# Funatiq/cuclark

Hardware: AMD Instinct MI355X
Metric: Mreads/sec (10M x 150bp, k=31) (higher is better)
Workload: dtype u64

## Files before the change

cuclark_amd/_lib.py:

```python
import ctypes as C
import importlib.util
import os
import subprocess

_PKG = os.path.dirname(os.path.abspath(__file__))
LIB_PATH = os.environ.get("MIC_LIB_PATH") or os.path.join(_PKG, "lib", "libmi_clark.so")
CSRC = os.path.join(_PKG, "csrc")

MIC_RESULT_WORDS = 8
MIC_FLAG_ROW_OVERFLOW = 1
MIC_FLAG_DENSE_PATH = 2
MIC_ROW_INVALID = 0xFFFFFFFF
MIC_ROLLUP_WORDS, MIC_ROLLUP_MAX_LEVELS = 8, 7
MIC_ROLLUP_UNRESOLVED, MIC_ROLLUP_PENDING = 0xFFFFFFFF, 0xFFFFFFFE
MIC_LAYOUT_AUTO, MIC_LAYOUT_DIRECT, MIC_LAYOUT_MINIMIZER, MIC_LAYOUT_SUPER, MIC_LAYOUT_SUPER2 = 0, 1, 2, 3, 4


class MicError(RuntimeError):
    def __init__(self, code, msg):
        super().__init__(f"libmi_clark error {code}: {msg}")
        self.code = code


class MicConfig(C.Structure):
    _fields_ = [("device", C.c_int32), ("k", C.c_int32), ("num_targets", C.c_uint32), ("num_batches", C.c_uint32),
                ("row_words", C.c_uint32), ("layout", C.c_uint32)]


class MicDbInfo(C.Structure):
    _fields_ = [("htsize", C.c_uint64), ("shard_start", C.c_uint64), ("shard_end", C.c_uint64),
                ("n_elems", C.c_uint64), ("n_elems_file", C.c_uint64), ("n_slots", C.c_uint64),
                ("n_overflow", C.c_uint64), ("hbm_bytes", C.c_uint64), ("key_bytes", C.c_int32),
                ("slot_class", C.c_int32), ("max_bucket", C.c_uint32), ("sampling", C.c_uint32), ("layout", C.c_int32),
                ("minimizer_len", C.c_int32), ("max_chain", C.c_uint32), ("reserved", C.c_uint32), ("n_entries", C.c_uint64),
                ("part", C.c_uint32), ("n_parts", C.c_uint32), ("part_slot_lo", C.c_uint64), ("part_slot_hi", C.c_uint64),
                ("n_slots_whole", C.c_uint64), ("side_kmers", C.c_uint64), ("side_bytes", C.c_uint64)]


class MicSynthSpec(C.Structure):
    _fields_ = [("seed", C.c_uint64), ("htsize", C.c_uint64), ("genome_nt", C.c_uint64), ("n_targets", C.c_uint32),
                ("n_genomes", C.c_uint32), ("k", C.c_int32), ("key_bytes", C.c_int32), ("keep_ppm", C.c_uint32), ("run_len", C.c_uint32),
                ("repeat_ppm", C.c_uint32), ("mosaic_ppm", C.c_uint32)]


class MicIngestResult(C.Structure):
    _fields_ = [("n_reads", C.c_uint64), ("csv_bytes", C.c_uint64), ("csv", C.c_void_p), ("results", C.c_void_p),
                ("status", C.c_uint32), ("n_lines", C.c_uint32)]


MIC_INGEST_OK, MIC_INGEST_FALLBACK, MIC_INGEST_ODD_RECORD, MIC_INGEST_TRUNCATED = 0, 1, 2, 4
MIC_INGEST_LONG_READ, MIC_INGEST_TOO_MANY, MIC_INGEST_DENSE = 8, 16, 32
MIC_INGEST_NO_CSV = 16


class MicAbundFilter(C.Structure):
    _fields_ = [("conf_num", C.c_uint64), ("conf_den", C.c_uint64), ("gamma_num", C.c_uint64), ("gamma_den", C.c_uint64)]

_VP, _SZ, _U32P, _U16P, _U64P = C.c_void_p, C.c_size_t, C.c_void_p, C.c_void_p, C.c_void_p
SYMBOLS = [
    ("mic_create", C.c_int, [C.POINTER(MicConfig), C.POINTER(_VP)]),
    ("mic_destroy", C.c_int, [_VP]),
    ("mic_last_error", C.c_char_p, []),
    ("mic_device_count", C.c_int, [C.POINTER(C.c_int)]),
    ("mic_db_load_files", C.c_int, [_VP, C.c_char_p, C.c_int, C.c_uint32, C.c_uint64, C.c_uint64]),
    ("mic_db_load_host", C.c_int, [_VP, _VP, C.c_uint64, _VP, C.c_int, _VP, C.c_uint32, C.c_uint64, C.c_uint64]),
    ("mic_db_load_device", C.c_int, [_VP, _VP, C.c_uint64, _VP, C.c_int, _VP, C.c_uint32, C.c_uint64, C.c_uint64]),
    ("mic_db_set_part", C.c_int, [_VP, C.c_uint32, C.c_uint32]),
    ("mic_db_reserve_hbm", C.c_int, [_VP, C.c_uint64]),
    ("mic_peer_matrix", C.c_int, [C.POINTER(C.c_int), C.c_int]),
    ("mic_device_memory", C.c_int, [C.c_int, C.POINTER(C.c_uint64), C.POINTER(C.c_uint64)]),
    ("mic_db_load_files_multi", C.c_int, [C.POINTER(C.c_void_p), _SZ, C.c_char_p, C.c_int, C.c_uint32]),
    ("mic_db_kernel_name", C.c_int, [_VP, C.c_char_p, _SZ]),
    ("mic_db_get_info", C.c_int, [_VP, C.POINTER(MicDbInfo)]),
    ("mic_db_unload", C.c_int, [_VP]),
    ("mic_db_last_build_report", C.c_char_p, []),
    ("mic_batches_alloc", C.c_int, [_VP, _SZ, _SZ, _SZ, _U32P, C.c_int, C.POINTER(_VP), C.POINTER(_VP), C.POINTER(_VP),
                                    C.POINTER(_VP)]),
    ("mic_batch_ready", C.c_int, [_VP, _SZ, _SZ, _SZ]),
    ("mic_batch_query", C.c_int, [_VP, _SZ, C.c_int, C.c_int]),
    ("mic_batch_wait", C.c_int, [_VP, _SZ]),
    ("mic_batch_dense_counts", C.c_int, [_VP, _SZ, _SZ, _VP]),
    ("mic_batch_check", C.c_int, [_VP, _SZ, C.POINTER(C.c_int)]),
    ("mic_batch_merge_shards", C.c_int, [C.POINTER(C.c_void_p), _SZ, _SZ]),
    ("mic_batch_query_group", C.c_int, [C.POINTER(C.c_void_p), _SZ, _SZ, C.c_int]),
    ("mic_sync", C.c_int, [_VP]),
    ("mic_thread_bind_near_device", C.c_int, [_VP, C.c_int]),
    ("mic_batches_free", C.c_int, [_VP]),
    ("mic_query_device", C.c_int, [_VP, _VP, _VP, _SZ, _VP, _VP, _VP]),
    ("mic_resolve_flagged_device", C.c_int, [_VP, _VP, _VP, _VP, _VP, _VP, C.POINTER(_SZ)]),
    ("mic_merge_rows_device", C.c_int, [_VP, _VP, _VP, _VP, _SZ, _VP]),
    ("mic_result_from_rows_device", C.c_int, [_VP, _VP, _VP, _SZ, _VP]),
    ("mic_count_dense_device", C.c_int, [_VP, _VP, _VP, _VP, _SZ, _VP, _VP]),
    ("mic_result_from_dense_device", C.c_int, [_VP, _VP, _VP, _SZ, _VP, _VP, _VP]),
    ("mic_probe_stats_device", C.c_int, [_VP, _VP, _VP, _SZ, C.POINTER(C.c_uint64)]),
    ("mic_last_query_ms", C.c_int, [_VP, C.POINTER(C.c_float)]),
    ("mic_last_crowd_stats", C.c_int, [_VP, C.POINTER(C.c_uint32)]),
    ("mic_debug_fetch_crowd", C.c_int, [_VP, _VP, _SZ, C.POINTER(C.c_uint32)]),
    ("mic_debug_stream_pool", C.c_int, [C.POINTER(C.c_uint32)]),
    ("mic_ingest_alloc", C.c_int, [_VP, _SZ, _SZ, C.POINTER(C.c_char_p), C.c_uint32, C.c_int, C.POINTER(_VP)]),
    ("mic_ingest_classify", C.c_int, [_VP, _SZ, _SZ, C.c_int, C.POINTER(MicIngestResult)]),
    ("mic_ingest_classify_group", C.c_int, [C.POINTER(C.c_void_p), _SZ, _SZ, _SZ, _SZ, C.c_int, C.POINTER(MicIngestResult)]),
    ("mic_ingest_fetch_group_rows", C.c_int, [_VP, _SZ, _SZ, _VP, _SZ, C.POINTER(C.c_uint64), C.POINTER(C.c_uint32)]),
    ("mic_ingest_group_stats", C.c_int, [_VP, C.POINTER(C.c_double), _SZ]),
    ("mic_ingest_fetch_packed", C.c_int, [_VP, _SZ, _VP, _SZ, _VP, _SZ, C.POINTER(C.c_uint64), C.POINTER(C.c_uint64)]),
    ("mic_ingest_free", C.c_int, [_VP]),
    ("mic_gz_inflate_device", C.c_int, [_VP, _VP, _SZ, C.POINTER(_VP), C.POINTER(_SZ), C.POINTER(C.c_uint32)]),
    ("mic_gz_copy_text", C.c_int, [_VP, _VP, _SZ, _SZ, _VP]),
    ("mic_gz_free_text", C.c_int, [_VP, _VP]),
    ("mic_gz_reserve", C.c_int, [_VP, _SZ, C.c_uint32]),
    ("mic_gz_reserve_bytes", C.c_uint64, [_SZ, C.c_uint32]),
    ("mic_gz_release", C.c_int, [_VP]),
    ("mic_pairs_index_device", C.c_int, [_VP, _VP, _SZ, _VP, _SZ, C.POINTER(_VP), C.POINTER(C.c_uint64), C.POINTER(C.c_uint32)]),
    ("mic_pairs_offsets", C.c_int, [_VP, C.POINTER(C.POINTER(C.c_uint64)), C.POINTER(_SZ), C.POINTER(C.c_uint32)]),
    ("mic_pairs_merge_to_slot", C.c_int, [_VP, _VP, C.c_uint64, C.c_uint64, _SZ, C.POINTER(_SZ)]),
    ("mic_pairs_text", C.c_int, [_VP, _VP, C.c_uint64, C.c_uint64, _VP, _SZ, C.POINTER(_SZ)]),
    ("mic_pairs_free", C.c_int, [_VP, _VP]),
    ("mic_text_index_device", C.c_int, [_VP, _VP, _SZ, C.POINTER(_VP), C.POINTER(C.c_uint64), C.POINTER(C.c_uint32)]),
    ("mic_text_index_front_device", C.c_int, [_VP, _VP, _SZ, C.POINTER(_VP), C.POINTER(C.c_uint64), C.POINTER(C.c_uint64), C.POINTER(C.c_uint32)]),
    ("mic_gz_stream_open", C.c_int, [_VP, _VP, _SZ, C.c_uint32, C.POINTER(_VP), C.POINTER(_VP), C.POINTER(_SZ)]),
    ("mic_gz_stream_next", C.c_int, [_VP, C.POINTER(_SZ), C.POINTER(C.c_int)]),
    ("mic_gz_stream_close", C.c_int, [_VP, C.c_int]),
    ("mic_text_offsets", C.c_int, [_VP, C.POINTER(C.POINTER(C.c_uint64)), C.POINTER(_SZ), C.POINTER(C.c_uint32)]),
    ("mic_text_to_slot", C.c_int, [_VP, _VP, C.c_uint64, C.c_uint64, _SZ, C.POINTER(_SZ)]),
    ("mic_text_copy", C.c_int, [_VP, _VP, C.c_uint64, C.c_uint64, _VP, _SZ, C.POINTER(_SZ)]),
    ("mic_text_free", C.c_int, [_VP, _VP]),
    ("mic_text_format", C.c_int, [_VP]),
    ("mic_abundance_start", C.c_int, [_VP, C.POINTER(MicAbundFilter)]),
    ("mic_abundance_fetch", C.c_int, [_VP, _VP, _SZ]),
    ("mic_abundance_stop", C.c_int, [_VP]),
    ("mic_abundance_device", C.c_int, [_VP, _VP, _VP, _SZ, C.POINTER(MicAbundFilter), _VP, _VP]),
    ("mic_abundance_host", C.c_int, [_VP, _VP, _SZ, C.c_int, C.c_uint32, C.POINTER(MicAbundFilter), _VP]),
    ("mic_abund_parse", C.c_int, [C.c_char_p, C.c_uint32, C.POINTER(C.c_uint64), C.POINTER(C.c_uint64)]),
    ("mic_rollup_check", C.c_int, [C.c_uint32, C.c_uint32, _VP]),
    ("mic_rollup_set", C.c_int, [_VP, C.c_uint32, _VP]),
    ("mic_rollup_layout", C.c_int, [_VP, _VP, C.POINTER(C.c_uint64)]),
    ("mic_rollup_device", C.c_int, [_VP, _VP, _VP, _SZ, C.POINTER(MicAbundFilter), _VP, _VP, _VP, _VP]),
    ("mic_rollup_dense_device", C.c_int, [_VP, _VP, _VP, _SZ, _VP, C.POINTER(MicAbundFilter), _VP, _VP, _VP, _VP]),
    ("mic_rollup_host", C.c_int, [_VP, C.c_uint32, _VP, _VP, _SZ, C.c_int, C.c_uint32, C.c_uint32, _VP, C.POINTER(MicAbundFilter),
                                  _VP, _VP, _VP]),
    ("mic_rollup_start", C.c_int, [_VP, C.POINTER(MicAbundFilter)]),
    ("mic_rollup_fetch", C.c_int, [_VP, _VP, _SZ]),
    ("mic_rollup_stop", C.c_int, [_VP]),
    ("mic_ingest_rollup_rows", C.c_int, [_VP, _SZ, C.POINTER(_VP), C.POINTER(C.c_uint64)]),
    ("mic_format_ratio_g", C.c_int, [C.c_uint32, C.c_uint32, C.c_char_p]),
    ("mic_key_bytes_rule", C.c_int, [C.c_uint64, C.c_int]),
    ("mic_index_reads", C.c_long, [_VP, _SZ, _SZ, _U64P, _U64P, _U64P, _U64P, _U64P]),
    ("mic_index_reads_parallel", C.c_long, [_VP, _SZ, C.c_int, _SZ, _U64P, _U64P, _U64P, _U64P, _U64P]),
    ("mic_find_record_start", _SZ, [_VP, _SZ, _SZ]),
    ("mic_find_record_start_in", _SZ, [_VP, _SZ, C.c_int, _SZ]),
    ("mic_pack_bound", _SZ, [_U64P, _U64P, _SZ, C.c_int]),
    ("mic_pack_reads", _SZ, [_VP, _U64P, _U64P, _U64P, _SZ, C.c_int, _U32P, _U16P, _SZ]),
    ("mic_csv_header", C.c_int, [C.c_char_p, _SZ, C.c_int, C.POINTER(C.c_char_p), C.c_uint32]),
    ("mic_csv_line", C.c_int, [C.c_char_p, _SZ, _VP, _SZ, C.c_uint64, C.c_int, C.c_int, _VP, C.POINTER(C.c_char_p),
                               C.c_uint32, C.c_int, _VP, _VP]),
    ("mic_db_build", C.c_int, [C.POINTER(C.c_char_p), _VP, _SZ, C.c_int, C.c_uint64, C.c_int, C.c_uint32, C.c_uint32, C.c_char_p,
                               C.c_int, C.c_int, C.c_uint32, C.POINTER(C.c_uint64)]),
    ("mic_db_build_error", C.c_char_p, []),
    ("mic_synth_db_device", C.c_int, [C.POINTER(MicSynthSpec), _VP, _VP, _VP, C.c_uint64, C.POINTER(C.c_uint64), _VP]),
    ("mic_synth_read_pitch", C.c_uint32, [C.c_uint32, C.c_int]),
    ("mic_synth_reads_device", C.c_int, [C.POINTER(MicSynthSpec), C.c_uint64, _SZ, C.c_uint32, C.c_double, C.c_double,
                                         C.c_double, _VP, _VP, _SZ, _VP, _VP]),
    ("mic_synth_reads_device2", C.c_int, [C.POINTER(MicSynthSpec), C.c_uint64, _SZ, C.c_uint32, C.c_int, C.c_double, C.c_double,
                                          C.c_double, _VP, _VP, _SZ, _VP, _VP]),
    ("mic_synth_text_record_bytes", _SZ, [C.c_uint32, C.c_int]),
    ("mic_synth_reads_text_device", C.c_int, [C.POINTER(MicSynthSpec), C.c_uint64, _SZ, C.c_uint32, C.c_double, C.c_double,
                                              C.c_double, C.c_int, C.c_int, _VP, _SZ, _VP]),
]

_lib = None


def build(verbose=False):
    r = subprocess.run(["make", "-C", CSRC, "all"], capture_output=True, text=True)
    if r.returncode != 0:
        raise RuntimeError("building libmi_clark.so failed:\n" + r.stdout[-4000:] + r.stderr[-4000:])
    if verbose:
        print(r.stdout)
    return LIB_PATH


def _share_hip_runtime_with_torch():
    if os.environ.get("MIC_NO_TORCH_HIP"):
        return
    try:
        spec = importlib.util.find_spec("torch")
    except Exception:
        spec = None
    if spec is None or not spec.origin:
        return
    p = os.path.join(os.path.dirname(spec.origin), "lib", "libamdhip64.so")
    if os.path.exists(p):
        try:
            C.CDLL(p, mode=C.RTLD_GLOBAL)
        except OSError:
            pass


def load():
    global _lib
    if _lib is not None:
        return _lib
    _share_hip_runtime_with_torch()
    if not os.path.exists(LIB_PATH):
        raise ImportError(f"{LIB_PATH} is missing: run `python -c 'import __graft_entry__ as g; g.build()'` "
                          "(there is no CPU fallback for the k-mer query path)")
    lib = C.CDLL(LIB_PATH)
    for name, res, args in SYMBOLS:
        fn = getattr(lib, name)
        fn.restype = res
        fn.argtypes = args
    _lib = lib
    return lib


def check(rc):
    if rc != 0:
        raise MicError(rc, load().mic_last_error().decode(errors="replace"))
```

cuclark_amd/csrc/mic_engine.hip:

```cpp
#include "mi_clark.h"
#include "mic_internal.h"

#include <errno.h>
#include <stdarg.h>
#include <stdio.h>
#include <stdlib.h>
#include <string.h>
#include <time.h>

#include <sched.h>

#include <algorithm>
#include <mutex>
#include <string>
#include <atomic>
#include <thread>
#include <unistd.h>
#include <utility>
#include <vector>

int mic_bind_thread_near_device(int device, int on);
bool mic_peer_enable(int from, int to);
void mic_peer_enable_engines(mic_engine* const* engines, size_t n);

// ... 36 lines not shown
  return he;
}

void mic_stream_put(hipStream_t s) {
  if (!s) return;
  (void)hipStreamSynchronize(s);
  StreamPool& P = pool();
  std::lock_guard<std::mutex> lk(P.mu);
  for (const auto& a : P.all_streams) if (a.second == s) { P.free_streams.push_back(a); return; }
}

hipError_t mic_event_get(hipEvent_t* ev, bool timing) {
  int dev = 0;
  hipError_t he = hipGetDevice(&dev);
  if (he != hipSuccess) return he;
  const int key = dev * 2 + (timing ? 1 : 0);
  StreamPool& P = pool();
  {
    std::lock_guard<std::mutex> lk(P.mu);
    for (size_t i = 0; i < P.free_events.size(); ++i)
      if (P.free_events[i].first == key) { *ev = P.free_events[i].second; P.free_events.erase(P.free_events.begin() + (ptrdiff_t)i); return hipSuccess; }
  }
  he = timing ? hipEventCreate(ev) : hipEventCreateWithFlags(ev, hipEventDisableTiming);
  if (he == hipSuccess) { std::lock_guard<std::mutex> lk(P.mu); P.all_events.emplace_back(key, *ev); }
  return he;
}

extern "C" int mic_debug_stream_pool(uint32_t out[4]) {
  if (!out) return MIC_E_INVALID;
  StreamPool& P = pool();
  std::lock_guard<std::mutex> lk(P.mu);
  out[0] = (uint32_t)P.all_streams.size(); out[1] = (uint32_t)P.free_streams.size();
  out[2] = (uint32_t)P.all_events.size(); out[3] = (uint32_t)P.free_events.size();
  return MIC_OK;
}

void mic_event_put(hipEvent_t ev) {
  if (!ev) return;
  (void)hipEventSynchronize(ev);
  StreamPool& P = pool();
  std::lock_guard<std::mutex> lk(P.mu);
  for (const auto& a : P.all_events) if (a.second == ev) { P.free_events.push_back(a); return; }
}
namespace {
std::mutex g_report_mu;
std::string g_report;
thread_local std::string t_report;

#define HIPTRY(x) do { hipError_t e_ = (x); if (e_ != hipSuccess) \
    return fail(e_ == hipErrorOutOfMemory ? MIC_E_NOMEM : MIC_E_HIP, "%s: %s", #x, hipGetErrorString(e_)); } while (0)

struct Batch {
  uint32_t* h_rp = nullptr; uint16_t* h_cont = nullptr;
  uint32_t* d_rp = nullptr; uint16_t* d_cont = nullptr;
  uint32_t* d_results = nullptr; uint32_t* d_rows = nullptr;
  uint32_t* d_flagged = nullptr; uint32_t* h_flagged = nullptr;
  uint32_t* d_peer = nullptr; uint32_t* d_acc = nullptr;
  uint32_t* d_crowd = nullptr;
  size_t first_read = 0, n_reads = 0, n_cont = 0, max_reads = 0, max_cont = 0;
  hipStream_t stream = nullptr;
  hipEvent_t done = nullptr, ev_up = nullptr, ev_k = nullptr;
  bool scheduled = false, resolved = true, extended = false;
};

}

struct mic_engine {
  mic_config cfg;
  int device = 0, n_cu = 256;
  hipStream_t stream = nullptr;
  hipStream_t up_stream = nullptr, down_stream = nullptr;
  bool db_loaded = false;
  uint4* slots = nullptr;
  uint4* side = nullptr;
  uint8_t* d_sizes = nullptr;
  MicTable table;
  int slot_class = 32;
  mic_db_info info;
  std::vector<Batch> batches;
  void* h_block = nullptr; void* d_block = nullptr;
  uint32_t* h_results = nullptr; uint32_t* h_rows = nullptr;
  size_t num_reads_total = 0;
  std::mutex submit_mu;
  uint32_t* d_flagged = nullptr; uint32_t flagged_cap = 0;
  uint32_t* d_crowd = nullptr; size_t crowd_reads = 0;
  hipEvent_t ev0 = nullptr, ev1 = nullptr;
  bool timed = false;
  size_t last_n_reads = 0;
  void* ingest = nullptr;
  uint64_t reserve_hbm = 0;
  uint32_t part = 0, n_parts = 0;
  MicAbund abund;
  MicRollup rollup;
};

namespace {

const uint32_t kFlaggedCap = 1u << 16;

int set_device(const mic_engine* e) {
  HIPTRY(hipSetDevice(e->device));
  return MIC_OK;
}

void fill_table(mic_engine* e, const MicBuildOut& b, uint64_t htsize, uint64_t s0, uint64_t s1, int key_bytes,
                uint32_t sampling, int layout, int m) {
  e->slots = b.slots;
  const bool parted = (layout == MIC_LAYOUT_SUPER || layout == MIC_LAYOUT_SUPER2) && (b.part_lo != 0 || b.part_hi != b.n_main);
  e->table.slots = parted ? b.slots - (ptrdiff_t)b.part_lo * 8 : b.slots;
  e->table.slot_lo = parted ? (uint32_t)b.part_lo : 0; e->table.slot_cnt = parted ? (uint32_t)(b.part_hi - b.part_lo) : 0;
  e->table.parted = parted ? 1 : 0;
  e->side = b.side;
  e->table.side = b.side; e->table.side_mask = b.side ? (uint32_t)(b.side_cells - 1) : 0;
  e->table.n_main = b.n_main;
  e->table.shard_start = s0;
  e->table.shard_end = s1;
  e->table.div = mic_make_div(htsize);
  e->table.k = e->cfg.k;
  e->table.layout = layout == MIC_LAYOUT_MINIMIZER ? 1 : (layout == MIC_LAYOUT_SUPER || layout == MIC_LAYOUT_SUPER2) ? 2 : 0;
  e->table.fwd = layout == MIC_LAYOUT_SUPER2 ? 1 : 0;
  e->table.m = m;
  e->table.sharded = (s0 != 0 || s1 != htsize) ? 1 : 0;
  e->table.sizes = e->d_sizes;
  mic_db_info& i = e->info;
  i.htsize = htsize; i.shard_start = s0; i.shard_end = s1;
  i.n_elems = b.n_elems; i.n_elems_file = b.n_elems_file;
  const uint64_t n_res = parted ? b.part_hi - b.part_lo : b.n_main;
  i.n_slots = n_res + b.n_overflow; i.n_overflow = b.n_overflow;
  i.part = e->n_parts > 1 ? e->part : 0; i.n_parts = e->n_parts > 1 ? e->n_parts : 0;
  i.part_slot_lo = parted ? b.part_lo : 0; i.part_slot_hi = parted ? b.part_hi : 0; i.n_slots_whole = b.n_main;
  i.side_kmers = b.side ? b.side_kmers : 0; i.side_bytes = b.side ? b.side_cells * 16 : 0;
  i.hbm_bytes = (b.side ? b.side_cells * 16 : 0) + (b.alloc_slots ? b.alloc_slots : n_res + b.n_overflow + 1) * (uint64_t)(layout != MIC_LAYOUT_DIRECT ? MIC_MSLOT_BYTES : MIC_SLOT_BYTES);
  i.key_bytes = key_bytes; i.slot_class = layout != MIC_LAYOUT_DIRECT ? 128 : e->slot_class; i.max_bucket = b.max_bucket;
  i.sampling = sampling; i.layout = layout; i.minimizer_len = layout != MIC_LAYOUT_DIRECT ? m : 0;
  i.max_chain = layout != MIC_LAYOUT_DIRECT ? b.max_chain : 0; i.reserved = (layout == MIC_LAYOUT_SUPER || layout == MIC_LAYOUT_SUPER2) ? b.walk_ppm : 0;
  i.n_entries = b.n_entries ? b.n_entries : b.n_elems;
  e->db_loaded = true;
  (void)mic_kernels_warm(e->stream);
}

int check_shard(uint64_t htsize, uint64_t& s0, uint64_t& s1) {
  if (htsize < 2 || htsize > 0xFFFFFFF0ULL) return fail(MIC_E_INVALID, "unsupported table size %llu", (unsigned long long)htsize);
  if (s1 == 0) s1 = htsize;
  if (s0 >= s1 || s1 > htsize) return fail(MIC_E_INVALID, "bad shard [%llu,%llu) of %llu", (unsigned long long)s0,
                                           (unsigned long long)s1, (unsigned long long)htsize);
  return MIC_OK;
}

struct UploadDst { int device; void* dst; hipStream_t stream; uint64_t lo, hi; };
struct UploadStage {
  static constexpr size_t CH = 256u << 20;
  void* buf[2] = {nullptr, nullptr};
  bool get(int near_device) {
    if (buf[0] && buf[1]) return true;
    mic_bind_thread_near_device(near_device, 1);
    bool ok = true;
    for (void*& b : buf) if (!b && ok) { ok = hipHostMalloc(&b, CH, hipHostMallocDefault) == hipSuccess; if (!ok) b = nullptr; }
    if (!ok) for (void*& b : buf) if (b) { hipHostFree(b); b = nullptr; }
    mic_bind_thread_near_device(near_device, 0);
    return ok;
  }
  ~UploadStage() { for (void* b : buf) if (b) hipHostFree(b); }
};
int upload_file_range_multi(FILE* f, const std::vector<UploadDst>& dsts, const char* what, UploadStage* shared = nullptr) {
  const size_t CH = UploadStage::CH;
  const int fd = fileno(f);
  static const int n_readers = [] { const char* e = getenv("MIC_LOAD_THREADS"); int v = e ? atoi(e) : 0; return v > 0 ? (v > 64 ? 64 : v) : 8; }();
// ... 327 lines not shown
void** mic_engine_ingest_slot(mic_engine* e) { return &e->ingest; }
MicAbund* mic_engine_abund(mic_engine* e) { return &e->abund; }
MicRollup* mic_engine_rollup(mic_engine* e) { return &e->rollup; }
uint32_t mic_engine_row_words(const mic_engine* e) { return e->cfg.row_words; }
hipStream_t mic_engine_stream(mic_engine* e) { return e->stream; }
void mic_engine_copy_streams(mic_engine* e, hipStream_t* up, hipStream_t* down) { *up = e->up_stream; *down = e->down_stream; }

void mic_build_report_add(const char* what, double seconds) {
  char line[256];
  snprintf(line, sizeof(line), "%s: %.4f\n", what, seconds);
  t_report += line;
}

namespace {
std::mutex g_peer_mu;
signed char g_peer[64][64];
}
bool mic_peer_enable(int from, int to) {
  if (from == to) return true;
  if (from < 0 || to < 0 || from >= 64 || to >= 64) return false;
  std::lock_guard<std::mutex> lk(g_peer_mu);
  if (g_peer[from][to]) return g_peer[from][to] > 0;
  int can = 0, cur = 0;
  hipGetDevice(&cur);
  bool ok = false;
  if (hipDeviceCanAccessPeer(&can, from, to) == hipSuccess && can && hipSetDevice(from) == hipSuccess) {
    const hipError_t he = hipDeviceEnablePeerAccess(to, 0);
    ok = he == hipSuccess || he == hipErrorPeerAccessAlreadyEnabled;
    (void)hipGetLastError();
  }
  hipSetDevice(cur);
  g_peer[from][to] = ok ? 1 : -1;
  return ok;
}
void mic_peer_enable_engines(mic_engine* const* engines, size_t n) {
  for (size_t i = 0; i < n; ++i)
    for (size_t j = 0; j < n; ++j)
      if (engines[i] && engines[j] && engines[i]->device != engines[j]->device) mic_peer_enable(engines[i]->device, engines[j]->device);
}

extern "C" {

const char* mic_last_error(void) { return g_err; }

int mic_device_count(int* count) {
  int n = 0;
  hipError_t e = hipGetDeviceCount(&n);
  if (e != hipSuccess) { *count = 0; return fail(MIC_E_NODEVICE, "hipGetDeviceCount: %s", hipGetErrorString(e)); }
  *count = n;
  return MIC_OK;
}

int mic_create(const mic_config* cfg, mic_engine** out) {
  if (!cfg || !out) return fail(MIC_E_INVALID, "null argument");
  if (cfg->k < 2 || cfg->k > 32) return fail(MIC_E_INVALID, "The k-mer length should be in [2,32].");
  if (cfg->num_targets > 65535) return fail(MIC_E_INVALID, "too many targets (%u > 65535)", cfg->num_targets);
  if (cfg->layout > MIC_LAYOUT_SUPER2) return fail(MIC_E_INVALID, "unknown table layout %u", cfg->layout);
  int n = 0;
  if (hipGetDeviceCount(&n) != hipSuccess || n == 0)
    return fail(MIC_E_NODEVICE, "no HIP device available: the MI355X engine cannot run (there is no CPU fallback)");
  int dev = cfg->device;
  if (dev < 0) { if (hipGetDevice(&dev) != hipSuccess) dev = 0; }
  if (dev >= n) return fail(MIC_E_INVALID, "device %d out of range (%d devices)", dev, n);
  hipDeviceProp_t prop;
  HIPTRY(hipSetDevice(dev));
  HIPTRY(hipGetDeviceProperties(&prop, dev));
  if (strncmp(prop.gcnArchName, "gfx950", 6) != 0)
    return fail(MIC_E_NODEVICE, "device %d is %s; this library carries gfx950 (MI355X) code objects only", dev, prop.gcnArchName);
  mic_engine* e = new (std::nothrow) mic_engine();
  if (!e) return fail(MIC_E_NOMEM, "out of host memory");
  e->cfg = *cfg;
  if (e->cfg.num_batches == 0) e->cfg.num_batches = 1;
  if (e->cfg.row_words == 0) e->cfg.row_words = 16;
  if (e->cfg.row_words < 2) e->cfg.row_words = 2;
  e->device = dev;
  e->n_cu = prop.multiProcessorCount;
  memset(&e->info, 0, sizeof(e->info));
  memset(&e->table, 0, sizeof(e->table));
  hipError_t he = mic_stream_get(&e->stream);
  if (he == hipSuccess) he = mic_stream_get(&e->up_stream);
  if (he == hipSuccess) he = mic_stream_get(&e->down_stream);
  if (he == hipSuccess) he = mic_event_get(&e->ev0, true);
  if (he == hipSuccess) he = mic_event_get(&e->ev1, true);
  if (he == hipSuccess) he = hipMalloc(&e->d_flagged, (size_t)(kFlaggedCap + 1) * 4);
  if (he != hipSuccess) { mic_destroy(e); return fail(MIC_E_HIP, "engine setup: %s", hipGetErrorString(he)); }
  e->flagged_cap = kFlaggedCap;
  *out = e;
  return MIC_OK;
}

int mic_destroy(mic_engine* e) {
  if (!e) return MIC_OK;
  hipSetDevice(e->device);
  hipDeviceSynchronize();
  mic_ingest_free(e);
  mic_gz_release(e);
  free_batches(e);
  if (e->slots) hipFree(e->slots);
  if (e->side) hipFree(e->side);
  if (e->d_sizes) hipFree(e->d_sizes);
  if (e->d_flagged) hipFree(e->d_flagged);
  if (e->d_crowd) hipFree(e->d_crowd);
  if (e->abund.d_counts) hipFree(e->abund.d_counts);
  if (e->rollup.d_counts) hipFree(e->rollup.d_counts);
  if (e->rollup.d_block) hipFree(e->rollup.d_block);
  if (e->ev0) mic_event_put(e->ev0);
  if (e->ev1) mic_event_put(e->ev1);
  if (e->stream) mic_stream_put(e->stream);
  if (e->up_stream) mic_stream_put(e->up_stream);
  if (e->down_stream) mic_stream_put(e->down_stream);
  delete e;
  return MIC_OK;
}

int mic_db_unload(mic_engine* e) {
  if (!e) return fail(MIC_E_INVALID, "null engine");
  int rc = set_device(e);
  if (rc) return rc;
  hipDeviceSynchronize();
  if (e->slots) hipFree(e->slots);
  if (e->side) hipFree(e->side);
  if (e->d_sizes) hipFree(e->d_sizes);
  e->slots = nullptr; e->side = nullptr; e->d_sizes = nullptr; e->db_loaded = false;
  memset(&e->info, 0, sizeof(e->info));
  return MIC_OK;
}

int mic_db_get_info(const mic_engine* e, mic_db_info* info) {
  if (!e || !info) return fail(MIC_E_INVALID, "null argument");
  if (!e->db_loaded) return fail(MIC_E_STATE, "no database loaded");
  *info = e->info;
  return MIC_OK;
}

const char* mic_db_last_build_report(void) {
  static thread_local std::string copy;
  std::lock_guard<std::mutex> lk(g_report_mu);
  copy = g_report;
  return copy.c_str();
}

int mic_db_reserve_hbm(mic_engine* e, uint64_t bytes) {
  if (!e) return fail(MIC_E_INVALID, "null engine");
  e->reserve_hbm = bytes;
  return MIC_OK;
}

int mic_db_set_part(mic_engine* e, uint32_t part, uint32_t n_parts) {
  if (!e) return fail(MIC_E_INVALID, "null engine");
  if (n_parts > 1 && part >= n_parts) return fail(MIC_E_INVALID, "part %u of %u", part, n_parts);
  if (n_parts > 65536) return fail(MIC_E_INVALID, "too many parts");
  if (e->db_loaded) return fail(MIC_E_STATE, "set the part before the database is loaded");
  e->part = n_parts > 1 ? part : 0; e->n_parts = n_parts > 1 ? n_parts : 0;
  return MIC_OK;
}

int mic_db_load_device(mic_engine* e, const uint8_t* d_sizes, uint64_t htsize, const void* d_keys, int key_bytes,
                       const uint16_t* d_labels, uint32_t sampling, uint64_t s0, uint64_t s1) {
  if (!e || !d_sizes || !d_keys || !d_labels) return fail(MIC_E_INVALID, "null argument");
  if (key_bytes != 2 && key_bytes != 4 && key_bytes != 8) return fail(MIC_E_INVALID, "key_bytes must be 2, 4 or 8");
  int rc = set_device(e);
  if (rc) return rc;
  if ((rc = check_shard(htsize, s0, s1))) return rc;
  if ((rc = apply_part(e, htsize, s0, s1))) return rc;
  if (e->db_loaded) mic_db_unload(e);
  uint64_t base_elems = 0, base_rank = 0;
  if (s0 > 0 && mic_reduce_sizes(d_sizes, s0, &base_elems, &base_rank, e->stream) != 0)
    return fail(MIC_E_HIP, "size reduction failed");
  return build_from_device(e, d_sizes + s0, htsize, s0, s1, (const char*)d_keys + base_elems * key_bytes, key_bytes,
                           d_labels + base_elems, sampling, base_rank);
}

int mic_db_load_host(mic_engine* e, const uint8_t* sizes, uint64_t htsize, const void* keys, int key_bytes,
                     const uint16_t* labels, uint32_t sampling, uint64_t s0, uint64_t s1) {
  if (!e || !sizes || !keys || !labels) return fail(MIC_E_INVALID, "null argument");
  if (key_bytes != 2 && key_bytes != 4 && key_bytes != 8) return fail(MIC_E_INVALID, "key_bytes must be 2, 4 or 8");
  int rc = set_device(e);
  if (rc) return rc;
  if ((rc = check_shard(htsize, s0, s1))) return rc;
  if ((rc = apply_part(e, htsize, s0, s1))) return rc;
  if (e->db_loaded) mic_db_unload(e);
  uint64_t base_elems = 0, base_rank = 0, n_el = 0;
  for (uint64_t i = 0; i < s0; ++i) { base_elems += sizes[i]; base_rank += sizes[i] > 0; }
  for (uint64_t i = s0; i < s1; ++i) n_el += sizes[i];
// ... 451 lines not shown
    std::vector<std::string> msgs(devs.size());
    std::vector<std::thread> th;
    for (size_t d = 0; d < devs.size(); ++d)
      th.emplace_back([&, d] {
        Dev& dv = devs[d];
        struct timespec ta; clock_gettime(CLOCK_MONOTONIC, &ta);
        for (size_t i : dv.eng) {
          mic_engine* e = engines[i];
          int r = set_device(e);
          if (!r) r = build_from_device(e, dv.d_sz + (er[i].s0 - dv.lo), htsize, er[i].s0, er[i].s1,
                                        (const char*)dv.d_ky + (er[i].base_elems - dv.el_lo) * key_bytes, key_bytes,
                                        dv.d_lb + (er[i].base_elems - dv.el_lo), sampling, er[i].base_rank);
          if (r) { rcs[d] = r; msgs[d] = g_err; break; }
        }
        hipSetDevice(dv.device);
        if (dv.d_sz) { hipFree(dv.d_sz); dv.d_sz = nullptr; }
        if (dv.d_ky) { hipFree(dv.d_ky); dv.d_ky = nullptr; }
        if (dv.d_lb) { hipFree(dv.d_lb); dv.d_lb = nullptr; }
        struct timespec tb; clock_gettime(CLOCK_MONOTONIC, &tb);
        dv.build_s = (tb.tv_sec - ta.tv_sec) + (tb.tv_nsec - ta.tv_nsec) / 1e9;
      });
    for (auto& t : th) t.join();
    for (size_t d = 0; d < devs.size(); ++d) if (rcs[d]) { rc = fail(rcs[d], "%s", msgs[d].c_str()); break; }
    if (timing)
      for (Dev& dv : devs) fprintf(stderr, "[load x%zu] device %d: %zu table(s) built in %.3f s\n", n_engines, dv.device, dv.eng.size(), dv.build_s);
    lap("tables built");
  } while (0);
  if (fs) fclose(fs);
  if (fk) fclose(fk);
  if (fl) fclose(fl);
  free(h_sz);
  for (Dev& dv : devs) {
    hipSetDevice(dv.device);
    if (dv.d_sz) hipFree(dv.d_sz);
    if (dv.d_ky) hipFree(dv.d_ky);
    if (dv.d_lb) hipFree(dv.d_lb);
  }
  return rc;
}

int mic_batch_check(mic_engine* e, size_t batch, int* done) {
  if (!e || batch >= e->batches.size() || !done) return fail(MIC_E_INVALID, "bad argument");
  Batch& B = e->batches[batch];
  if (!B.scheduled) { *done = 0; return MIC_OK; }
  hipError_t he = hipEventQuery(B.done);
  if (he == hipSuccess) *done = 1;
  else if (he == hipErrorNotReady) *done = 0;
  else return fail(MIC_E_HIP, "hipEventQuery: %s", hipGetErrorString(he));
  return MIC_OK;
}

int mic_thread_bind_near_device(mic_engine* e, int on) {
  if (!e) return fail(MIC_E_INVALID, "null engine");
  mic_bind_thread_near_device(e->device, on);
  return MIC_OK;
}

int mic_sync(mic_engine* e) {
  if (!e) return fail(MIC_E_INVALID, "null engine");
  int rc = set_device(e);
  if (rc) return rc;
  HIPTRY(hipDeviceSynchronize());
  return MIC_OK;
}

int mic_batches_free(mic_engine* e) {
  if (!e) return fail(MIC_E_INVALID, "null engine");
  int rc = set_device(e);
  if (rc) return rc;
  hipDeviceSynchronize();
  free_batches(e);
  return MIC_OK;
}

int mic_query_device(mic_engine* e, const uint32_t* d_rp, const uint16_t* d_cont, size_t n_reads, uint32_t* d_results,
                     uint32_t* d_rows, void* stream) {
  if (!e || !d_rp || !d_cont || !d_results) return fail(MIC_E_INVALID, "null argument");
  if (!e->db_loaded) return fail(MIC_E_STATE, "no database loaded");
  if (n_reads > 0xFFFFFFF0ull) return fail(MIC_E_INVALID, "too many reads in one call");
  if (((uintptr_t)d_cont & 3) || ((uintptr_t)d_rp & 3)) return fail(MIC_E_INVALID, "d_containers and d_reads_pointer must be 4-byte aligned");
  int rc = set_device(e);
  if (rc) return rc;
  hipStream_t s = stream ? (hipStream_t)stream : e->stream;
  HIPTRY(hipMemsetAsync(e->d_flagged, 0, 4, s));
  MicQueryArgs a;
  a.t = e->table; a.reads_ptr = d_rp; a.cont = d_cont; a.n_reads = (uint32_t)n_reads;
  a.row_words = e->cfg.row_words; a.results = d_results; a.rows = d_rows;
  a.flagged = e->d_flagged; a.flagged_cap = e->flagged_cap;
  if (e->table.side && n_reads > e->crowd_reads) {
    HIPTRY(hipStreamSynchronize(s));
    if (e->d_crowd) { hipFree(e->d_crowd); e->d_crowd = nullptr; e->crowd_reads = 0; }
    HIPTRY(hipMalloc(&e->d_crowd, mic_crowd_dims(n_reads).words * 4));
    e->crowd_reads = n_reads;
  }
  mic_crowd_attach(a, e->table.side ? e->d_crowd : nullptr, e->crowd_reads);
  HIPTRY(hipEventRecord(e->ev0, s));
  HIPTRY(mic_launch_query(a, e->slot_class, e->n_cu, s));
  HIPTRY(hipEventRecord(e->ev1, s));
  e->timed = true;
  e->last_n_reads = n_reads;
  return MIC_OK;
}

int mic_last_query_ms(mic_engine* e, float* ms) {
  if (!e || !ms) return fail(MIC_E_INVALID, "null argument");
  if (!e->timed) return fail(MIC_E_STATE, "no query was launched");
  HIPTRY(hipEventSynchronize(e->ev1));
  HIPTRY(hipEventElapsedTime(ms, e->ev0, e->ev1));
  return MIC_OK;
}

int mic_last_crowd_stats(mic_engine* e, uint32_t out[4]) {
  if (!e || !out) return fail(MIC_E_INVALID, "null argument");
  out[0] = out[1] = out[2] = out[3] = 0;
  if (!e->timed || !e->d_crowd || !e->table.side) return MIC_OK;
  int rc = set_device(e);
  if (rc) return rc;
  HIPTRY(hipEventSynchronize(e->ev1));
  HIPTRY(hipMemcpy(out, e->d_crowd, 16, hipMemcpyDeviceToHost));
  return MIC_OK;
}

int mic_debug_fetch_crowd(mic_engine* e, uint32_t* out, size_t words, uint32_t caps[3]) {
  if (!e || !out || !caps) return fail(MIC_E_INVALID, "null argument");
  if (!e->d_crowd || !e->timed) return fail(MIC_E_STATE, "no work area");
  int rc = set_device(e);
  if (rc) return rc;
  const MicCrowdDims d = mic_crowd_dims(e->crowd_reads);
  caps[0] = d.pend_cap; caps[1] = d.item_cap; caps[2] = d.pool_cap;
  HIPTRY(hipEventSynchronize(e->ev1));
  HIPTRY(hipMemcpy(out, e->d_crowd, (words < d.words ? words : d.words) * 4, hipMemcpyDeviceToHost));
  return MIC_OK;
}

int mic_resolve_flagged_device(mic_engine* e, const uint32_t* d_rp, const uint16_t* d_cont, uint32_t* d_results,
                               uint32_t* d_rows, void* stream, size_t* n_resolved) {
  if (!e || !d_rp || !d_cont || !d_results) return fail(MIC_E_INVALID, "null argument");
  int rc = set_device(e);
  if (rc) return rc;
  hipStream_t s = stream ? (hipStream_t)stream : e->stream;
  uint32_t nf = 0;
  HIPTRY(hipMemcpyAsync(&nf, e->d_flagged, 4, hipMemcpyDeviceToHost, s));
  HIPTRY(hipStreamSynchronize(s));
  if (n_resolved) *n_resolved = nf;
  if (!nf) return MIC_OK;
  if (nf > e->flagged_cap) {
    if (n_resolved) *n_resolved = e->last_n_reads;
    return run_dense(e, d_rp, d_cont, nullptr, e->last_n_reads, d_results, d_rows, s);
  }
  return run_dense(e, d_rp, d_cont, e->d_flagged + 1, nf, d_results, d_rows, s);
}

int mic_merge_rows_device(mic_engine* e, const uint32_t* a, const uint32_t* b, uint32_t* out, size_t n, void* stream) {
  if (!e || !a || !b || !out) return fail(MIC_E_INVALID, "null argument");
  int rc = set_device(e);
  if (rc) return rc;
  HIPTRY(mic_launch_merge_rows(a, b, out, e->cfg.row_words, n, nullptr, stream ? (hipStream_t)stream : e->stream));
  return MIC_OK;
}

int mic_result_from_rows_device(mic_engine* e, const uint32_t* rows, uint32_t* results, size_t n, void* stream) {
  if (!e || !rows || !results) return fail(MIC_E_INVALID, "null argument");
  int rc = set_device(e);
  if (rc) return rc;
  HIPTRY(mic_launch_result_from_rows(rows, e->cfg.row_words, results, n, stream ? (hipStream_t)stream : e->stream));
  return MIC_OK;
}

int mic_result_from_dense_device(mic_engine* e, const uint32_t* d_counts, const uint32_t* d_ids, size_t n_ids, uint32_t* d_results,
                                 uint32_t* d_rows, void* stream) {
  if (!e || !d_counts || !d_results) return fail(MIC_E_INVALID, "null argument");
  int rc = set_device(e);
  if (rc) return rc;
  HIPTRY(mic_launch_dense_finish(d_counts, d_ids, n_ids, e->cfg.num_targets ? e->cfg.num_targets : 1, d_results, d_rows,
                                 e->cfg.row_words, stream ? (hipStream_t)stream : e->stream));
  return MIC_OK;
}

int mic_probe_stats_device(mic_engine* e, const uint32_t* d_rp, const uint16_t* d_cont, size_t n_reads, uint64_t out[4]) {
  if (!e || !d_rp || !d_cont || !out) return fail(MIC_E_INVALID, "null argument");
  if (!e->db_loaded) return fail(MIC_E_STATE, "no database loaded");
  int rc = set_device(e);
  if (rc) return rc;
  unsigned long long* d = nullptr;
  unsigned long long h[4] = {0, 0, 0, 0};
  HIPTRY(hipMalloc(&d, 32));
  hipError_t he = hipMemsetAsync(d, 0, 32, e->stream);
  if (he == hipSuccess) he = mic_launch_probe_stats(e->table, e->slot_class, d_rp, d_cont, n_reads, d, e->stream);
  if (he == hipSuccess) he = hipMemcpyAsync(h, d, 32, hipMemcpyDeviceToHost, e->stream);
  if (he == hipSuccess) he = hipStreamSynchronize(e->stream);
  hipFree(d);
  if (he != hipSuccess) return fail(MIC_E_HIP, "probe stats: %s", hipGetErrorString(he));
  for (int i = 0; i < 4; ++i) out[i] = h[i];
  return MIC_OK;
}

int mic_count_dense_device(mic_engine* e, const uint32_t* d_rp, const uint16_t* d_cont, const uint32_t* d_ids,
                           size_t n_ids, uint32_t* d_counts, void* stream) {
  if (!e || !d_rp || !d_cont || !d_counts) return fail(MIC_E_INVALID, "null argument");
  if (!e->db_loaded) return fail(MIC_E_STATE, "no database loaded");
  int rc = set_device(e);
  if (rc) return rc;
// ... 7 lines not shown
```

cuclark_amd/csrc/mic_internal.h:

```cpp
#ifndef MIC_INTERNAL_H
#define MIC_INTERNAL_H

#include <hip/hip_runtime.h>
#include <stdint.h>
#include <stddef.h>

#include "mi_clark.h"

struct MicDiv {
  uint64_t d;
  uint64_t magic;
  uint32_t shift;
  uint32_t add;
};

MicDiv mic_make_div(uint64_t d);

#ifdef __cplusplus
#include <vector>
size_t mic_pack_reads_runs(const uint8_t* map, const uint64_t* seq_s, const uint64_t* seq_e, const uint64_t* length,
                           size_t n_reads, int k, uint32_t* reads_pointer, uint16_t* containers, size_t cap,
                           std::vector<uint64_t>* run_off, std::vector<uint64_t>* run_len);
#endif

static inline __host__ __device__ uint64_t mic_mulhi64(uint64_t a, uint64_t b) {
#if defined(__HIP_DEVICE_COMPILE__)
  return __umul64hi(a, b);
#else
  return (uint64_t)(((unsigned __int128)a * b) >> 64);
#endif
}

static inline __host__ __device__ uint64_t mic_div(uint64_t n, const MicDiv& dv) {
  if (dv.magic == 0) return n >> dv.shift;
  uint64_t t = mic_mulhi64(dv.magic, n);
  if (dv.add) return (((n - t) >> 1) + t) >> dv.shift;
  return t >> dv.shift;
}

#define MIC_SLOT_BYTES 64
#define MIC_FLAG_ROW_OVERFLOW_ 1u
#define MIC_FLAG_DENSE_PATH_ 2u
#define MIC_ROW_INVALID 0xFFFFFFFFu
#define MIC_CAP32 8
#define MIC_CAP64 4

#define MIC_MCAP 12
#define MIC_MSLOT_BYTES 128
#ifndef MIC_LAYOUT_MINIMIZER
#define MIC_LAYOUT_AUTO 0
#define MIC_LAYOUT_DIRECT 1
#define MIC_LAYOUT_MINIMIZER 2
#endif
#ifndef MIC_LAYOUT_SUPER
#define MIC_LAYOUT_SUPER 3
#endif
#ifndef MIC_LAYOUT_SUPER2
#define MIC_LAYOUT_SUPER2 4
#endif

struct MicTable {
  const uint4* slots;
  uint64_t n_main;
  uint64_t shard_start;
  uint64_t shard_end;
  MicDiv div;
  int k;
  int layout;
  int m;
  int sharded;
  int fwd;
  uint32_t slot_lo, slot_cnt;
  const uint4* side; uint32_t side_mask;
  int parted;
  const uint8_t* sizes;
};

struct MicQueryArgs {
  MicTable t;
  const uint32_t* reads_ptr;
  const uint16_t* cont;
  uint32_t n_reads;
  uint32_t row_words;
  uint32_t* results;
  uint32_t* rows;
  uint32_t* flagged;
  uint32_t flagged_cap;
  uint32_t* crowd;
  uint32_t* crowd_items; uint32_t* crowd_pool;
  uint32_t crowd_pend_cap, crowd_item_cap, crowd_pool_cap;
};

#define MIC_CROWD_HDR 8
#define MIC_CG_NONE 0xFFFFFFFFu
#define MIC_CG_DENSE 0xFFFFFFFEu
struct MicCrowdDims { uint32_t pend_cap, item_cap, pool_cap; size_t words; };
static inline MicCrowdDims mic_crowd_dims(size_t max_reads) {
  MicCrowdDims d;
  const size_t cap27 = (1u << 27) - 64;
  size_t pend = max_reads / 4 + 1024, item = max_reads + 4096, pool = max_reads * 2 + 8192;
  d.pend_cap = (uint32_t)(pend < cap27 ? pend : cap27);
  d.item_cap = (uint32_t)(item < cap27 ? item : cap27);
  d.pool_cap = (uint32_t)(pool < 0xFFFFFF00u ? pool : 0xFFFFFF00u);
  d.words = MIC_CROWD_HDR + 8 * ((size_t)d.pend_cap + d.item_cap) + d.pool_cap;
  return d;
}
static inline void mic_crowd_attach(MicQueryArgs& a, uint32_t* area, size_t max_reads) {
  const MicCrowdDims d = mic_crowd_dims(max_reads);
  a.crowd = area; a.crowd_pend_cap = area ? d.pend_cap : 0; a.crowd_item_cap = area ? d.item_cap : 0; a.crowd_pool_cap = area ? d.pool_cap : 0;
  a.crowd_items = area ? area + MIC_CROWD_HDR + 8 * (size_t)d.pend_cap : nullptr;
  a.crowd_pool = area ? a.crowd_items + 8 * (size_t)d.item_cap : nullptr;
}

void mic_build_report_add(const char* what, double seconds);
extern thread_local uint64_t mic_build_reserved_hbm;

hipError_t mic_launch_query(const MicQueryArgs& a, int slot_class, int n_cu, hipStream_t s);
int mic_query_kernel_name(const MicTable& t, int slot_class, char* buf, size_t cap);
hipError_t mic_kernels_warm(hipStream_t s);
hipError_t mic_launch_merge_rows(const uint32_t* a, const uint32_t* b, uint32_t* out, uint32_t row_words, size_t n,
                                 uint32_t* flags_results, hipStream_t s);
hipError_t mic_launch_result_from_rows(const uint32_t* rows, uint32_t row_words, uint32_t* results, size_t n,
                                       hipStream_t s);
hipError_t mic_launch_dense_count(const MicTable& t, int slot_class, const uint32_t* reads_ptr, const uint16_t* cont,
                                  const uint32_t* ids, size_t n_ids, uint32_t n_targets, uint32_t* counts,
                                  hipStream_t s);
hipError_t mic_launch_dense_finish(const uint32_t* counts, const uint32_t* ids, size_t n_ids, uint32_t n_targets,
                                   uint32_t* results, uint32_t* rows, uint32_t row_words, hipStream_t s);

hipError_t mic_launch_probe_stats(const MicTable& t, int slot_class, const uint32_t* reads_ptr, const uint16_t* cont,
                                  size_t n_reads, unsigned long long* d_out, hipStream_t s);

struct MicBuildOut {
  uint4* slots;
  uint64_t n_main, n_overflow, n_elems, n_elems_file;
  uint32_t max_bucket;
  uint32_t max_chain;
  uint32_t walk_ppm;
  uint64_t n_entries;
  uint4* side; uint64_t side_cells, side_kmers;
  uint64_t part_lo, part_hi;
  uint64_t alloc_slots;
};
int mic_build_table(const uint8_t* d_sizes, uint64_t n_buckets, const void* d_keys, int key_bytes,
                    const uint16_t* d_labels, uint32_t sampling, uint64_t rank_base, int slot_class, hipStream_t s,
                    MicBuildOut* out, char* err, size_t err_cap);
int mic_build_mtable(const uint8_t* d_sizes, uint64_t n_buckets, uint64_t bucket0, uint64_t htsize, const void* d_keys,
                     int key_bytes, const uint16_t* d_labels, uint32_t sampling, uint64_t rank_base, int k, int m,
                     hipStream_t s, MicBuildOut* out, char* err, size_t err_cap);
int mic_build_stable(const uint8_t* d_sizes, uint64_t n_buckets, uint64_t bucket0, uint64_t htsize, const void* d_keys,
                     int key_bytes, const uint16_t* d_labels, uint32_t sampling, uint64_t rank_base, int k, int m,
                     hipStream_t s, MicBuildOut* out, char* err, size_t err_cap, int allow_fallback, int both_strands,
                     uint32_t part, uint32_t n_parts);
int mic_reduce_sizes(const uint8_t* d_sizes, uint64_t n, uint64_t* total, uint64_t* nonzero, hipStream_t s);

hipError_t mic_stream_get(hipStream_t* s);
void mic_stream_put(hipStream_t s);
hipError_t mic_event_get(hipEvent_t* ev, bool timing);
void mic_event_put(hipEvent_t ev);

struct MicAbund {
  unsigned long long* d_counts = nullptr;
  uint32_t n_words = 0;
  bool on = false;
  uint64_t conf_num = 5, conf_den = 10, gamma_num = 0, gamma_den = 1;
};
hipError_t mic_launch_abund(const uint32_t* results, const uint32_t* norm, uint32_t norm_sub, size_t n, int k, uint32_t n_targets,
                            const MicAbund& f, unsigned long long* counts, const uint32_t* status, hipStream_t s);

struct MicRollup {
  uint32_t n_levels = 0;
  uint32_t n_groups[8] = {};
  uint32_t off[8] = {};
  uint32_t seg_off[8] = {};
  uint32_t n_counters = 0;
  void* d_block = nullptr;
  const uint16_t* d_group_of = nullptr;
  const uint16_t* d_perm = nullptr;
  const uint32_t* d_seg = nullptr;
  unsigned long long* d_counts = nullptr;
  bool on = false;
  mic_abund_filter filter = {5, 10, 0, 1};
};
hipError_t mic_launch_rollup(const MicRollup& ru, const uint32_t* rows, uint32_t row_words, const uint32_t* norm, uint32_t norm_sub, size_t n,
                             int k, uint32_t n_targets, const mic_abund_filter& f, uint32_t* rollup, uint32_t* levels,
                             unsigned long long* counts, const uint32_t* status, hipStream_t s);

#endif
```

cuclark_amd/csrc/mic_kernels.hip:

```cpp
#include "mic_internal.h"
#include "mic_device.h"

#include <stdlib.h>

#ifndef MIC_EXP
#define MIC_EXP 0
#endif
#ifndef MIC_FUNNEL64
#define MIC_FUNNEL64 1
#endif
#ifndef MIC_X
#define MIC_X 0
#endif

namespace {

__device__ __forceinline__ uint4 load_slot_quarter(const uint4* p) {
  typedef unsigned int u4 __attribute__((ext_vector_type(4)));
  u4 t = __builtin_nontemporal_load((const u4*)p);
  return make_uint4(t.x, t.y, t.z, t.w);
}

__device__ __forceinline__ uint64_t kmer_from_dwords(uint32_t d0, uint32_t d1, uint32_t d2, int nt_in_dword, int k) {
  const int s = 2 * nt_in_dword;
  uint64_t a = ((uint64_t)d0 << 32) | d1;
#if MIC_FUNNEL64
  uint64_t x = (a << s) | ((uint64_t)d2 >> (32 - s));
#else
  uint64_t x = s ? ((a << s) | (uint64_t)(d2 >> (32 - s))) : a;
#endif
  return x >> (64 - 2 * k);
}


struct ReadAhead { uint32_t pp, pe, hdr, w; };

__device__ __forceinline__ void ahead_ptr(const MicQueryArgs& a, uint32_t r, ReadAhead& x) {
  if (r < a.n_reads) { x.pp = a.reads_ptr[r]; x.pe = a.reads_ptr[r + 1]; } else { x.pp = 0; x.pe = 0; }
}

__device__ __forceinline__ void ahead_window(const uint16_t* __restrict__ cont, uint32_t r, uint32_t n_reads, int lane,
                                             ReadAhead& x) {
  x.hdr = 0; x.w = 0;
  if (r < n_reads) {
    const uint32_t pp = __builtin_amdgcn_readfirstlane(x.pp);
    x.hdr = cont[pp];
    if (lane < 10) x.w = ((uint32_t)cont[pp + 1 + 2 * lane] << 16) | cont[pp + 2 + 2 * lane];
  }
}

__device__ __forceinline__ uint32_t window_word(const uint16_t* __restrict__ cont, uint32_t first, uint32_t cend,
                                                uint32_t base, int lane, bool use_ahead, const ReadAhead& x) {
  uint32_t w = 0;
  const uint32_t ci = first + base / 8 + 2 * lane;
  if (use_ahead) w = x.w;
  else if (lane < 10) w = ((ci < cend ? (uint32_t)cont[ci] : 0u) << 16) | (ci + 1 < cend ? (uint32_t)cont[ci + 1] : 0u);
  if (lane >= 10 || ci >= cend) w &= 0x0000FFFFu;
  if (lane >= 10 || ci + 1 >= cend) w &= 0xFFFF0000u;
  return w;
}

__device__ __forceinline__ uint32_t window_word_w(const uint16_t* __restrict__ cont, uint32_t first, uint32_t cend,
                                                  uint32_t base, int lane, bool use_ahead, uint32_t ahead_w) {
  uint32_t w = 0;
  const uint32_t ci = first + base / 8 + 2 * lane;
  if (use_ahead) w = ahead_w;
  else if (lane < 10) w = ((ci < cend ? (uint32_t)cont[ci] : 0u) << 16) | (ci + 1 < cend ? (uint32_t)cont[ci + 1] : 0u);
  if (lane >= 10 || ci >= cend) w &= 0x0000FFFFu;
  if (lane >= 10 || ci + 1 >= cend) w &= 0xFFFF0000u;
  return w;
}

struct Probe {
  uint32_t slot;
  uint32_t qlo, qhi;
};

template <bool KEY64>
__device__ __forceinline__ Probe make_probe(const MicTable& t, uint64_t kmer, bool active) {
  uint64_t c = canonical(kmer, t.k);
  uint64_t q = mic_div(c, t.div);
  uint64_t rem = c - q * t.div.d;
  Probe p;
  bool ok = active && rem >= t.shard_start && rem < t.shard_end;
  if (!KEY64) ok = ok && (q >> 32) == 0;
  p.slot = ok ? (uint32_t)(rem - t.shard_start) : 0xFFFFFFFFu;
// ... 146 lines not shown
    }
  }
}

template <bool KEY64>
__global__ void __launch_bounds__(256) query_kernel(const MicQueryArgs a) {
  const int lane = threadIdx.x & 63;
  const int j = lane & 3;
  const uint32_t wave0 = __builtin_amdgcn_readfirstlane(blockIdx.x * 4 + (threadIdx.x >> 6));
  const uint32_t n_waves = gridDim.x * 4;
  const MicTable& t = a.t;
  const int k = t.k;
  const uint4* __restrict__ slots = t.slots;
  const uint16_t* __restrict__ cont = a.cont;

  for (uint32_t r = wave0; r < a.n_reads; r += n_waves) {
    ReadAhead cur;
    ahead_ptr(a, r, cur);
    ahead_window(cont, r, a.n_reads, lane, cur);
    uint32_t pp = __builtin_amdgcn_readfirstlane(cur.pp);
    const uint32_t pe = __builtin_amdgcn_readfirstlane(cur.pe);
    RowAcc acc; acc.label1 = 0; acc.count = 0;
    uint32_t n_ent = 0, overflow = 0, total = 0;
    bool first_part = true;

    while (pp < pe) {
      const uint32_t plen = __builtin_amdgcn_readfirstlane(first_part ? cur.hdr : (uint32_t)cont[pp]);
      const bool ahead_ok = first_part;
      first_part = false;
      if (plen == 0) break;
      const uint32_t first = pp + 1;
      pp = first + (plen + 7) / 8;
      if (plen < (uint32_t)k) continue;
      const uint32_t nk = plen - k + 1;
      const uint32_t cend = pp;
      for (uint32_t base = 0; base < nk; base += 128) {
        const uint32_t w = window_word(cont, first, cend, base, lane, ahead_ok && base == 0, cur);
        Probe pr[2];
#pragma unroll
        for (int h = 0; h < 2; ++h) {
          const int idx = 4 * h + (lane >> 4);
          uint32_t d0 = bperm(idx, w), d1 = bperm(idx + 1, w), d2 = bperm(idx + 2, w);
          uint64_t kmer = kmer_from_dwords(d0, d1, d2, lane & 15, k);
          pr[h] = make_probe<KEY64>(t, kmer, base + 64 * h + lane < nk);
        }
        uint4 q[8]; uint32_t qlo[8], qhi[8]; uint32_t sl[8];
#pragma unroll
        for (int s = 0; s < 8; ++s) {
          const int src = 16 * (s & 3) + (lane >> 2);
          sl[s] = bperm(src, pr[s >> 2].slot);
          qlo[s] = bperm(src, pr[s >> 2].qlo);
          qhi[s] = KEY64 ? bperm(src, pr[s >> 2].qhi) : 0;
          q[s] = make_uint4(0, 0, 0, 0);
          if (sl[s] != 0xFFFFFFFFu) q[s] = load_slot_quarter(slots + (uint64_t)sl[s] * 4 + j);
        }
        uint32_t res0 = 0, res1 = 0;
#pragma unroll
        for (int s = 0; s < 8; ++s) {
          uint32_t m = match_quarter<KEY64>(q[s], qlo[s], qhi[s], j);
          m |= quad_perm<QP_XOR1>(m);
          m |= quad_perm<QP_XOR2>(m);
          constexpr uint32_t CAP = KEY64 ? MIC_CAP64 : MIC_CAP32;
          if (__ballot((q[s].w & 0xFF) > CAP))
            m = chase_chain<KEY64>(slots, q[s], qlo[s], qhi[s], j, m, sl[s] != 0xFFFFFFFFu);
          if (s < 4) res0 = (j == (s & 3)) ? m : res0;
          else res1 = (j == (s & 3)) ? m : res1;
        }
        tally2(res0, res1, acc, n_ent, overflow, total, lane);
      }
    }
    finish_read(acc, n_ent, total, overflow, r, a, lane);
  }
}


#define MIC_RMAX 32
#define MIC_MSTRIDE 8
#ifndef MIC_R_SKEW
#define MIC_R_SKEW 2
#endif
#ifndef MIC_R_PIPE
#define MIC_R_PIPE 2
#endif
__device__ __forceinline__ uint32_t staged_at(uint32_t i) { return i * MIC_MSTRIDE + (i >> 3) * MIC_R_SKEW; }
#ifndef MIC_M_SKEW
#define MIC_M_SKEW 0
#endif
__device__ __forceinline__ uint32_t staged_at_m(uint32_t i) { return i * MIC_MSTRIDE + (i >> 3) * MIC_M_SKEW; }

__device__ __forceinline__ void sliding_min3(uint32_t& a0, uint32_t& a1, uint32_t& a2, int w, int lane) {
  auto step = [&](int s) {
    const int src = (lane + s) & 63;
    const bool wrap = lane + s >= 64;
    uint32_t x0 = bperm(src, a0), x1 = bperm(src, a1), x2 = bperm(src, a2);
    uint32_t n0 = wrap ? x1 : x0, n1 = wrap ? x2 : x1, n2 = wrap ? 0xFFFFFFFFu : x2;
    a0 = n0 < a0 ? n0 : a0; a1 = n1 < a1 ? n1 : a1; a2 = n2 < a2 ? n2 : a2;
  };
  int cover = 1;
  while (2 * cover <= w) { step(cover); cover *= 2; }
  if (cover < w) step(w - cover);
}

__device__ __forceinline__ void sliding_min2(uint32_t& a0, uint32_t& a1, int w, int lane) {
  auto step = [&](int s) {
    const int src = (lane + s) & 63;
    const bool wrap = lane + s >= 64;
    uint32_t x0 = bperm(src, a0), x1 = bperm(src, a1);
    uint32_t n0 = wrap ? x1 : x0, n1 = wrap ? 0xFFFFFFFFu : x1;
    a0 = n0 < a0 ? n0 : a0; a1 = n1 < a1 ? n1 : a1;
  };
  int cover = 1;
  while (2 * cover <= w) { step(cover); cover *= 2; }
  if (cover < w) step(w - cover);
}

__device__ __forceinline__ uint32_t row_prefix_min(uint32_t t) {
  uint32_t x;
  x = (uint32_t)__builtin_amdgcn_update_dpp(-1, (int)t, 0x111, 0xF, 0xF, false); t = x < t ? x : t;
  x = (uint32_t)__builtin_amdgcn_update_dpp(-1, (int)t, 0x112, 0xF, 0xF, false); t = x < t ? x : t;
  x = (uint32_t)__builtin_amdgcn_update_dpp(-1, (int)t, 0x114, 0xF, 0xF, false); t = x < t ? x : t;
  x = (uint32_t)__builtin_amdgcn_update_dpp(-1, (int)t, 0x118, 0xF, 0xF, false); t = x < t ? x : t;
  return t;
}

__device__ __forceinline__ uint32_t row_suffix_min(uint32_t t) {
  uint32_t x;
  x = (uint32_t)__builtin_amdgcn_update_dpp(-1, (int)t, 0x101, 0xF, 0xF, false); t = x < t ? x : t;
  x = (uint32_t)__builtin_amdgcn_update_dpp(-1, (int)t, 0x102, 0xF, 0xF, false); t = x < t ? x : t;
  x = (uint32_t)__builtin_amdgcn_update_dpp(-1, (int)t, 0x104, 0xF, 0xF, false); t = x < t ? x : t;
  x = (uint32_t)__builtin_amdgcn_update_dpp(-1, (int)t, 0x108, 0xF, 0xF, false); t = x < t ? x : t;
  return t;
}

template <int BANKS>
__device__ __forceinline__ uint32_t with_row_in_front(uint32_t P) {
  const uint32_t f = (uint32_t)__builtin_amdgcn_update_dpp(-1, (int)P, 0x142, 0xE, BANKS, false);
  return f < P ? f : P;
}
__device__ __forceinline__ void sliding_min_rows(uint32_t& a0, uint32_t& a1, uint32_t a2, int W, int lane, int lane_inv) {
  const uint32_t P0 = row_prefix_min(a0), P1 = row_prefix_min(a1), P2 = row_prefix_min(a2);
  if (W > 16 && ((W - 16) & 3) == 0) {
    const uint32_t S0 = row_suffix_min(a0), S1 = row_suffix_min(a1);
    const int s = W - 16, bm = (1 << (s >> 2)) - 1;
    uint32_t Q0, Q1, Q2;
    switch (bm) {
      case 1: Q0 = with_row_in_front<1>(P0); Q1 = with_row_in_front<1>(P1); Q2 = with_row_in_front<1>(P2); break;
      case 3: Q0 = with_row_in_front<3>(P0); Q1 = with_row_in_front<3>(P1); Q2 = with_row_in_front<3>(P2); break;
      case 7: Q0 = with_row_in_front<7>(P0); Q1 = with_row_in_front<7>(P1); Q2 = with_row_in_front<7>(P2); break;
      default: Q0 = with_row_in_front<15>(P0); Q1 = with_row_in_front<15>(P1); Q2 = with_row_in_front<15>(P2); break;
    }
    const uint32_t f0 = __builtin_amdgcn_readlane(P0, 63), f1 = __builtin_amdgcn_readlane(P1, 63);
    const bool head = lane < s;
    const uint32_t h1 = f0 < Q1 ? f0 : Q1, h2 = f1 < Q2 ? f1 : Q2;
    Q1 = head ? h1 : Q1; Q2 = head ? h2 : Q2;
    const int at = (lane_inv << 2) + ((W - 1) << 2);
    const uint32_t z0 = (uint32_t)__builtin_amdgcn_ds_bpermute(at, (int)Q0), z1 = (uint32_t)__builtin_amdgcn_ds_bpermute(at, (int)Q1),
                   z2 = (uint32_t)__builtin_amdgcn_ds_bpermute(at, (int)Q2);
    const bool wz = lane >= 65 - W;
    const uint32_t v0 = wz ? z1 : z0, v1 = wz ? z2 : z1;
    a0 = v0 < S0 ? v0 : S0; a1 = v1 < S1 ? v1 : S1;
    return;
  }
  const uint32_t S0 = row_suffix_min(a0), S1 = row_suffix_min(a1), S2 = row_suffix_min(a2);
  const int at = lane_inv << 2;
  const uint32_t x0 = (uint32_t)__builtin_amdgcn_ds_bpermute(at + 60, (int)P0), x1 = (uint32_t)__builtin_amdgcn_ds_bpermute(at + 60, (int)P1),
                 x2 = (uint32_t)__builtin_amdgcn_ds_bpermute(at + 60, (int)P2);
// ... 506 lines not shown
                const bool m1 = same1 && ((p1 >> (16 + (w - 1) - ao[1])) & 1) && s_extract(a1, b1, c1, (int)ao[1], k) == ko[1];
                if (m0) hit0 = (p0 & 0xFFFFu) + 1;
                if (m1) hit1 = (p1 & 0xFFFFu) + 1;
                {
                  const bool cr0 = same0 && (p0 >> 16) == 0, cr1 = same1 && (p1 >> 16) == 0;
                  if (__ballot(cr0) | __ballot(cr1)) {
                    uint64_t kp = (uint64_t)__builtin_amdgcn_kernarg_segment_ptr();
                    asm volatile("" : "+s"(kp));
                    const __attribute__((address_space(4))) MicQueryArgs* kc = (const __attribute__((address_space(4))) MicQueryArgs*)kp;
                    const uint4* side = kc->t.side; const uint32_t smask = kc->t.side_mask;
                    const uint64_t mm = (1ULL << (2 * m)) - 1;
                    if (side && cr0 && s_extract(a0, b0, c0, w - 1, m) == ((ko[0] >> (2 * ao[0])) & mm)) hit0 = s_side_probe(side, smask, ko[0]);
                    if (side && cr1 && s_extract(a1, b1, c1, w - 1, m) == ((ko[1] >> (2 * ao[1])) & mm)) hit1 = s_side_probe(side, smask, ko[1]);
                  }
                }
                more0 = same0 && !m0 && e0 < 5; more1 = same1 && !m1 && e1 < 5;
                e0 += more0 ? 1u : 0u; e1 += more1 ? 1u : 0u;
                if (!(__ballot(more0) | __ballot(more1))) break;
              }
              if (v0) { o0_ = hit0; y0_ = 0xFFFFFFFFu; }
              if (v1) { o1_ = hit1; y1_ = 0xFFFFFFFFu; }
              const bool n0 = v0 && !hit0 && (mz0 & MIC_S_NEXT), n1 = v1 && !hit1 && (mz1 & MIC_S_NEXT);
              if (__ballot(n0) | __ballot(n1)) {
                if (n0 && q0[5] <= t0) y0_ = q0[31];
                if (n1 && q1[5] <= t1) y1_ = q1[31];
              }
            }
          }
        };
        while (__ballot(sl0 != 0xFFFFFFFFu) | __ballot(sl1 != 0xFFFFFFFFu)) {
          uint32_t nx0, nx1;
          level(sl0, sl1, res0, res1, nx0, nx1);
          sl0 = nx0; sl1 = nx1;
        }
        tally2(res0, res1, acc, n_ent, overflow, total, lane);
      }
    }
    uint32_t t_hdr, t_pp, t_pe;
    asm volatile("s_waitcnt vmcnt(0)" ::: "memory");
    __builtin_amdgcn_wave_barrier();
    ahead_take(ahead_sel ? ahead1 : ahead0, n_pp, t_hdr, t_pp, t_pe);
    __builtin_amdgcn_wave_barrier();
    {
      uint64_t kp = (uint64_t)__builtin_amdgcn_kernarg_segment_ptr();
      asm volatile("" : "+s"(kp));
      const __attribute__((address_space(4))) MicQueryArgs* kc = (const __attribute__((address_space(4))) MicQueryArgs*)kp;
      struct { uint32_t* results; uint32_t* rows; uint32_t* flagged; uint32_t row_words, flagged_cap; } fa;
      fa.results = kc->results; fa.rows = kc->rows; fa.flagged = kc->flagged; fa.row_words = kc->row_words; fa.flagged_cap = kc->flagged_cap;
      finish_read(acc, n_ent, total, overflow, r, fa, lane);
    }
    ahead_issue(ahead_sel ? ahead0 : ahead1, t_pp, r + 3 * n_waves);
    ahead_sel ^= 1;
    cur_pp = n_pp; cur_pe = n_pe; cur_hdr = t_hdr; n_pp = t_pp; n_pe = t_pe;
  }
}


__device__ __forceinline__ uint64_t wballot(bool p) { return __builtin_amdgcn_ballot_w64(p); }

static_assert(MIC_RMAX <= 32, "tally_counts sums the first two rows of lanes");
#define MIC_R_CROWDED (-16)
__device__ __forceinline__ void tally_counts(uint32_t lab1, uint32_t cnt, RowAcc& acc, uint32_t& n_ent, uint32_t& overflow,
                                             uint32_t& total, int lane) {
  uint64_t mm = wballot(lab1 != 0);
  while (mm) {
    const uint32_t l1 = __builtin_amdgcn_readlane(lab1, __builtin_ctzll(mm));
    const bool mine = lab1 == l1;
    mm &= ~wballot(mine);
    const uint32_t c = mine ? cnt : 0u;
    uint32_t sum = 0;
    {
      uint32_t v = c;
      v += (uint32_t)__builtin_amdgcn_update_dpp(0, (int)v, 0x111, 0xF, 0xF, true);
      v += (uint32_t)__builtin_amdgcn_update_dpp(0, (int)v, 0x112, 0xF, 0xF, true);
      v += (uint32_t)__builtin_amdgcn_update_dpp(0, (int)v, 0x114, 0xF, 0xF, true);
      v += (uint32_t)__builtin_amdgcn_update_dpp(0, (int)v, 0x118, 0xF, 0xF, true);
      sum = __builtin_amdgcn_readlane(v, 15) + __builtin_amdgcn_readlane(v, 31);
    }
    total += sum;
    row_add(acc, n_ent, overflow, l1, sum, lane);
  }
}

template <int KK, int MM, bool FWD, bool PART>
__global__ void __launch_bounds__(64 * MIC_M_WPB, 32 / MIC_M_WPB) query_kernel_r(const MicQueryArgs a) {
  __shared__ uint4 s_stage[MIC_M_WPB][MIC_RMAX * MIC_MSTRIDE + (MIC_RMAX / 8 - 1) * MIC_R_SKEW];
  __shared__ uint16_t s_rec[MIC_M_WPB][132];
  __shared__ uint32_t s_ahead[MIC_M_WPB][2][64];
  __shared__ uint32_t s_part[PART ? MIC_M_WPB : 1][2];
  const int lane = threadIdx.x & 63;
  const int wv = __builtin_amdgcn_readfirstlane(threadIdx.x >> 6);
  uint4* stage = s_stage[wv];
  uint16_t* rec = s_rec[wv];
  const uint32_t wave0 = __builtin_amdgcn_readfirstlane(blockIdx.x * MIC_M_WPB + wv);
  const uint32_t n_waves = gridDim.x * MIC_M_WPB;
  const MicTable& t = a.t;
  if (PART) { if (lane == 0) { s_part[wv][0] = t.slot_lo; s_part[wv][1] = t.slot_cnt; } __builtin_amdgcn_wave_barrier(); }
  const int k = KK ? KK : t.k, m = MM ? MM : t.m, ctx = k - m;
  const uint4* __restrict__ slots = t.slots;
  const uint16_t* __restrict__ cont = a.cont;
  auto below = [](uint64_t mask) { return (uint32_t)__builtin_amdgcn_mbcnt_hi((uint32_t)(mask >> 32), __builtin_amdgcn_mbcnt_lo((uint32_t)mask, 0u)); };

  uint32_t* ahead0 = s_ahead[wv][0];
  uint32_t* ahead1 = s_ahead[wv][1];
  auto ahead_issue = [&](uint32_t* entry, uint32_t pp_w, uint32_t r_ptr) {
    const uint64_t abase = ((uint64_t)(cont + pp_w)) & ~3ULL;
    const uint32_t rr = r_ptr < a.n_reads ? r_ptr : a.n_reads - 1;
    const uint64_t pbase = (uint64_t)(a.reads_ptr + rr) - 48;
    int ln = lane;
    asm volatile("" : "+v"(ln));
    if (ln < 12)
      __builtin_amdgcn_global_load_lds((const __attribute__((address_space(1))) void*)((const uint32_t*)abase + lane),
                                       (__attribute__((address_space(3))) void*)entry, 4, 0, 0);
    uint64_t pb = pbase + 48;
    asm volatile("" : "+s"(pb));
    if (ln < 2)
      __builtin_amdgcn_global_load_lds((const __attribute__((address_space(1))) void*)((const uint32_t*)pb + lane),
                                       (__attribute__((address_space(3))) void*)(entry + 12), 4, 0, 0);
  };
  auto ahead_take = [&](const uint32_t* entry, uint32_t pp_w, uint32_t& hdr, uint32_t& npp, uint32_t& npe) {
    const uint32_t raw = entry[lane];
    npp = __builtin_amdgcn_readlane(raw, 12); npe = __builtin_amdgcn_readlane(raw, 13);
    const bool odd = (((uint64_t)(cont + pp_w)) >> 1) & 1;
    const uint32_t first = __builtin_amdgcn_readfirstlane(raw);
    hdr = odd ? first >> 16 : first & 0xFFFFu;
  };
  auto ahead_word = [&](const uint32_t* entry, uint32_t pp_w) {
    const uint32_t raw = entry[lane];
    const bool odd = (((uint64_t)(cont + pp_w)) >> 1) & 1;
    const uint32_t up = (uint32_t)__builtin_amdgcn_update_dpp(0, (int)raw, 0x101, 0xF, 0xF, true);
    return __builtin_amdgcn_perm(up, raw, odd ? 0x05040706u : 0x03020504u);
  };
  uint32_t cur_pp, cur_pe, cur_hdr, n_pp, n_pe, ahead_sel;
  {
    const uint32_t r0 = wave0 < a.n_reads ? wave0 : a.n_reads - 1;
    cur_pp = __builtin_amdgcn_readfirstlane(a.reads_ptr[r0]); cur_pe = __builtin_amdgcn_readfirstlane(a.reads_ptr[r0 + 1]);
    ahead_issue(ahead0, cur_pp, wave0 + n_waves);
    asm volatile("s_waitcnt vmcnt(0)" ::: "memory");
    __builtin_amdgcn_wave_barrier();
    ahead_take(ahead0, cur_pp, cur_hdr, n_pp, n_pe);
    ahead_issue(ahead1, n_pp, wave0 + 2 * n_waves);
    ahead_sel = 1;
  }
  constexpr bool PIPE = KK != 0 && (MIC_R_PIPE >= 2 || (MIC_R_PIPE == 1 && FWD));
  struct Round {
    uint32_t G0, G1, G2, cur;
    int jmax, jmin, remaining;
  };
  auto front = [&](const uint32_t first, const uint32_t cend, const uint32_t base, const uint32_t nk, const bool use_ahead, uint32_t& wd_out) __attribute__((always_inline)) -> uint32_t {
    int ln = lane;
    asm volatile("" : "+v"(ln));
    const uint32_t wd = use_ahead ? ahead_word(ahead_sel ? ahead0 : ahead1, cur_pp)
                                  : window_word_w(cont, first, cend, base, ln, false, 0u);
    wd_out = wd;
    const uint32_t n_act = nk - base < 128u ? nk - base : 128u;
    const bool past = n_act + (uint32_t)(k - s_tlen(k, m)) >= 129u;
    uint32_t qa0, qa1;
    sampled_positions<!FWD>(wd, ln, lane, k, m, past, qa0, qa1);
    qa0 = (uint32_t)lane < n_act ? qa0 : 0xFFu;
    qa1 = 64u + (uint32_t)lane < n_act ? qa1 : 0xFFu;
    const uint32_t last0 = __builtin_amdgcn_readlane(qa0, 63);
    uint32_t p0 = (uint32_t)__builtin_amdgcn_update_dpp(-1, (int)qa0, 0x138, 0xF, 0xF, false);
    uint32_t p1 = (uint32_t)__builtin_amdgcn_update_dpp((int)last0, (int)qa1, 0x138, 0xF, 0xF, false);
    const bool f0 = qa0 != p0, f1 = qa1 != p1;
    const uint64_t b0 = wballot(f0), b1 = wballot(f1);
    const uint32_t R0 = __popcll(b0), R = R0 + __popcll(b1) - (n_act < 128u ? 1u : 0u);
    __builtin_amdgcn_wave_barrier();
    if (f0) rec[below(b0)] = (uint16_t)(qa0 | ((uint32_t)lane << 8));
    if (f1) rec[R0 + below(b1)] = (uint16_t)(qa1 | ((64u + (uint32_t)lane) << 8));
    if (__builtin_expect(n_act == 128u, 0)) {
      asm volatile("" ::: "memory");
      if (ln == 0) rec[R] = (uint16_t)(128u << 8);
    }
    __builtin_amdgcn_wave_barrier();
    return R;
  };
  const uint32_t xsh = (64u - 2u * (uint32_t)k) & 31u;
  auto region_x = [&](uint32_t A0, uint32_t A1, uint32_t& lo, uint32_t& hi) {
    if (k > 16) {
      lo = __builtin_amdgcn_alignbit(A0, A1, xsh) & (m >= 16 ? 0xFFFFFFFFu : (1u << ((2 * m) & 31)) - 1u);
      hi = m > 16 ? (A0 >> xsh) & ((1u << ((2 * m - 32) & 31)) - 1u) : 0u;
    } else {
      const uint64_t x = ((((uint64_t)A0 << 32) | A1) << (2 * ctx)) >> (64 - 2 * m);
      lo = (uint32_t)x; hi = (uint32_t)(x >> 32);
    }
  };
  auto setup = [&](const uint32_t wd, const uint32_t rbase, const uint32_t R, Round& L, uint32_t& nrun_out) __attribute__((always_inline)) {
    const uint32_t nrun = R - rbase < MIC_RMAX ? R - rbase : MIC_RMAX;
    nrun_out = nrun;
    const bool vr = (uint32_t)lane < nrun;
    const uint32_t ri = vr ? rbase + (uint32_t)lane : 0u;
    const uint32_t rc0 = rec[ri], rc1 = rec[ri + 1];
    const int qa = (int)(rc0 & 255u), i0 = (int)(rc0 >> 8);
    const int n = (int)(rc1 >> 8) - i0;
    const int s1 = qa - ctx - 1;
    const int D = s1 >> 4;
    const uint32_t tsh = 30u - 2u * (uint32_t)(s1 & 15);
    const int a0 = D << 2;
    const uint32_t W0 = (uint32_t)__builtin_amdgcn_ds_bpermute(a0, (int)wd), W1 = (uint32_t)__builtin_amdgcn_ds_bpermute(a0 + 4, (int)wd),
                   W2 = (uint32_t)__builtin_amdgcn_ds_bpermute(a0 + 8, (int)wd), W3 = (uint32_t)__builtin_amdgcn_ds_bpermute(a0 + 12, (int)wd);
    uint32_t G0 = __builtin_amdgcn_alignbit(W0, W1, tsh), G1 = __builtin_amdgcn_alignbit(W1, W2, tsh), G2 = __builtin_amdgcn_alignbit(W2, W3, tsh);
    uint32_t key, xhi;
    region_x(G0, G1, key, xhi);
    bool rev = false;
    if (!FWD) {
      const uint32_t sh = 96u - 2u * (uint32_t)(k + ctx);
      const uint32_t r0 = __builtin_bitreverse32(G2), r1 = __builtin_bitreverse32(G1), r2 = __builtin_bitreverse32(G0);
      uint32_t q0 = sh ? __builtin_amdgcn_alignbit(r0, r1, 32u - sh) : r0;
      uint32_t q1 = sh ? __builtin_amdgcn_alignbit(r1, r2, 32u - sh) : r1;
      uint32_t q2 = r2 << sh;
      q0 = ~(((q0 >> 1) & 0x55555555u) | ((q0 << 1) & 0xAAAAAAAAu));
      q1 = ~(((q1 >> 1) & 0x55555555u) | ((q1 << 1) & 0xAAAAAAAAu));
      q2 = ~(((q2 >> 1) & 0x55555555u) | ((q2 << 1) & 0xAAAAAAAAu));
      uint32_t kr, hr;
      region_x(q0, q1, kr, hr);
      rev = hr < xhi || (hr == xhi && kr < key);
      G0 = rev ? q0 : G0; G1 = rev ? q1 : G1; G2 = rev ? q2 : G2;
      key = rev ? kr : key; xhi = rev ? hr : xhi;
    }
    const int jmaxf = qa - i0, jminf = jmaxf - n + 1;
    const int jmax = rev ? ctx - jminf : jmaxf, jmin = rev ? ctx - jmaxf : jminf;
    uint32_t cur = vr ? sslot_of_x32(key, xhi, (uint32_t)t.n_main) : 0xFFFFFFFFu;
    bool mine = vr;
    if (PART) {
      mine = vr && cur - s_part[wv][0] < s_part[wv][1];
      cur = mine ? cur : 0xFFFFFFFFu;
    }
    L.G0 = G0; L.G1 = G1; L.G2 = G2; L.cur = cur;
    L.jmax = jmax; L.jmin = jmin; L.remaining = mine ? n : 0;
  };
  auto issue = [&](const uint32_t cur, const uint32_t nrun) __attribute__((always_inline)) {
    uint32_t sidx[MIC_RMAX / 8];
    int ln = lane;
    asm volatile("" : "+v"(ln));
    __builtin_amdgcn_wave_barrier();
    if (ln < MIC_RMAX) ((uint32_t*)stage)[lane] = cur;
    __builtin_amdgcn_wave_barrier();
    uint32_t so = (uint32_t)(uintptr_t)(__attribute__((address_space(3))) void*)stage;
    asm volatile("" : "+s"(so));
#pragma unroll
    for (int i = 0; i < MIC_RMAX / 8; ++i) sidx[i] = ((const uint32_t*)stage)[8 * i + (lane >> 3)];
#pragma unroll
    for (int i = 0; i < MIC_RMAX / 8; ++i) {
      if (8u * i >= nrun) break;
      if (sidx[i] != 0xFFFFFFFFu)
        __builtin_amdgcn_global_load_lds((const __attribute__((address_space(1))) void*)(slots + (uint64_t)sidx[i] * 8 + (lane & 7)),
                                         (__attribute__((address_space(3))) void*)(uintptr_t)(so + 16u * (64 + MIC_R_SKEW) * (uint32_t)i), 16, 0, 0);
    }
  };
  auto consume = [&](Round& L, RowAcc& acc, uint32_t& n_ent, uint32_t& overflow, uint32_t& total, uint32_t& cg) __attribute__((always_inline)) {
    const uint32_t G0 = L.G0, G1 = L.G1, G2 = L.G2;
    uint32_t key, xhi_;
    region_x(G0, G1, key, xhi_);
    const int jmax = L.jmax, jmin = L.jmin;
    uint32_t cur = L.cur;
    int remaining = L.remaining;
    bool again = false;
    do {
      if (again) issue(cur, MIC_RMAX);
      again = true;
      asm volatile("s_waitcnt vmcnt(0)" ::: "memory");
      __builtin_amdgcn_wave_barrier();
      const bool vl = cur != 0xFFFFFFFFu;
      const uint32_t* q = (const uint32_t*)(stage + (vl ? staged_at((uint32_t)lane) : 0));
      const uint4 ka = *(const uint4*)q;
      const uint2 kb = *(const uint2*)(q + 4);
      uint32_t e = (ka.x < key) + (ka.y < key) + (ka.z < key) + (ka.w < key) + (kb.x < key) + (kb.y < key);
      const uint32_t mz = q[30];
      bool more = vl && e < 6;
      e = e < 5 ? e : 5;
      for (;;) {
        uint32_t e3 = e + (e << 1);
        asm volatile("" : "+v"(e3));
        uint32_t g = q[e], S0 = q[6 + e3], S1 = q[7 + e3], S2 = q[8 + e3], pl = q[24 + e];
        asm volatile("" : "+v"(S2));
        const bool same = more && g == key;
        const uint32_t d0 = G0 ^ S0, d1 = G1 ^ S1, d2 = G2 ^ S2;
        const bool mineq = k > 16
                               ? ((d0 & ((1u << ((32 - 2 * ctx) & 31)) - 1u)) | (d1 >> xsh)) == 0
                               : (((((uint64_t)d0 << 32) | d1) << (2 * ctx)) >> (64 - 2 * m)) == 0;
        const uint32_t dl = d0 >> (32 - 2 * ctx);
        const uint32_t dr = k > 16 ? __builtin_amdgcn_alignbit(d1, d2, xsh)
                                        : (uint32_t)((((((uint64_t)d0 << 32) | d1)) << ((2 * k) & 63)) >> 32);
        const int left = __builtin_ctz(dl | (1u << (2 * ctx))) >> 1;
        const int right = __builtin_clz(dr | (1u << (31 - 2 * ctx))) >> 1;
        const int hi = left < jmax ? left : jmax, lo = ctx - right > jmin ? ctx - right : jmin;
        const uint32_t range = ((2u << (hi & 31)) - 1u) & (~0u << (lo & 31));
        const uint32_t hits = (same && mineq) ? (uint32_t)__popc((pl >> 16) & range) : 0u;
#if !(MIC_X & 1)
        remaining = (same && mineq && (pl >> 16) == 0) ? MIC_R_CROWDED : remaining;
#endif
        const uint32_t lab_new = (pl & 0xFFFFu) + 1u;
        tally_counts(hits ? lab_new : 0u, hits, acc, n_ent, overflow, total, lane);
        remaining -= (int)hits;
        more = same && remaining > 0 && e < 5;
        e += more ? 1u : 0u;
        if (!wballot(more)) break;
      }
      const bool nx = vl && remaining > 0 && (mz & MIC_S_NEXT);
      cur = 0xFFFFFFFFu;
      if (wballot(nx)) { if (nx && q[5] <= key) cur = q[31]; }
    } while (wballot(cur != 0xFFFFFFFFu));
    if (!(MIC_X & 2) && __builtin_expect(wballot(remaining <= MIC_R_CROWDED) != 0, 0)) {
      const bool crowded = remaining <= MIC_R_CROWDED;
      const uint32_t n_c = (uint32_t)__popcll(wballot(crowded));
      uint64_t kpv = (uint64_t)__builtin_amdgcn_kernarg_segment_ptr();
      asm volatile("" : "+v"(kpv));
      const MicQueryArgs* kv = (const MicQueryArgs*)kpv;
      uint32_t* cw = kv->crowd;
      uint32_t* itb = kv->crowd_items;
      const uint32_t icap = kv->crowd_item_cap;
      uint32_t ib = 0xFFFFFFFFu;
      if (cw != nullptr && cg != MIC_CG_DENSE) {
        uint32_t v = 0;
        if (lane == 0) v = atomicAdd(&cw[1], n_c);
        ib = __builtin_amdgcn_readfirstlane(v);
      }
      asm volatile("" : "+v"(ib));
      const bool room = ib <= icap && n_c <= icap - ib;
      if (crowded && room) {
        uint32_t* it = itb + 8 * ((size_t)ib + below(wballot(crowded)));
        it[0] = G0; it[1] = G1; it[2] = G2; it[3] = (uint32_t)jmin | ((uint32_t)jmax << 8);
        it[4] = cg;
      }
      cg = __builtin_amdgcn_readfirstlane(room ? (ib | ((n_c - 1u) << 27)) : MIC_CG_DENSE);
    }
  };
  auto finish = [&](const RowAcc& acc, uint32_t n_ent, uint32_t total, uint32_t overflow, uint32_t r, const uint32_t cg) __attribute__((always_inline)) {
    uint32_t spilled = 0;
    if (!(MIC_X & 4) && __builtin_expect(cg != MIC_CG_NONE, 0)) {
      uint64_t kpv = (uint64_t)__builtin_amdgcn_kernarg_segment_ptr();
      asm volatile("" : "+v"(kpv));
      const MicQueryArgs* kv = (const MicQueryArgs*)kpv;
      uint32_t* cw = kv->crowd;
      uint32_t* pool = kv->crowd_pool;
      const uint32_t pcap = kv->crowd_pend_cap, wcap = kv->crowd_pool_cap;
      uint32_t p = 0xFFFFFFFFu, off = 0;
      if (cg != MIC_CG_DENSE) {
        if (lane == 0) { p = atomicAdd(&cw[0], 1u); off = atomicAdd(&cw[2], 2u * n_ent); }
        p = __builtin_amdgcn_readfirstlane(p); off = __builtin_amdgcn_readfirstlane(off);
      }
      asm volatile("" : "+v"(p), "+v"(off));
      const bool room = off <= wcap && 2u * n_ent <= wcap - off;
      if (p < pcap) {
        uint32_t* pd = cw + MIC_CROWD_HDR + 8 * (size_t)p;
        if (lane == 0) { pd[0] = r; pd[1] = total; pd[2] = room ? (n_ent | (overflow << 8)) : 0xFFFFFFFFu; pd[3] = off; pd[4] = cg; }
        if (room && (uint32_t)lane < n_ent) { uint32_t* pe_ = pool + (size_t)off + 2 * lane; pe_[0] = acc.label1; pe_[1] = acc.count; }
      }
      spilled = __builtin_amdgcn_readfirstlane((p < pcap && room) ? 1u : 0u);
      if (!spilled) {
        if (lane == 0 && cw != nullptr && cg != MIC_CG_DENSE) atomicAdd(&cw[3], 1u);
        overflow = 1;
      }
    }
    if (!spilled) {
      uint64_t kp = (uint64_t)__builtin_amdgcn_kernarg_segment_ptr();
      asm volatile("" : "+s"(kp));
      const __attribute__((address_space(4))) MicQueryArgs* kc = (const __attribute__((address_space(4))) MicQueryArgs*)kp;
      struct { uint32_t* results; uint32_t* rows; uint32_t* flagged; uint32_t row_words, flagged_cap; } fa;
      fa.results = kc->results; fa.rows = kc->rows; fa.flagged = kc->flagged; fa.row_words = kc->row_words; fa.flagged_cap = kc->flagged_cap;
      finish_read(acc, n_ent, total, overflow, r, fa, lane);
    }
  };

  uint32_t r = wave0; bool p_valid = false;
  auto step = [&](Round& P, Round& N) __attribute__((always_inline)) -> bool {
    const bool have = r < a.n_reads;
    uint32_t pp = cur_pp;
    const uint32_t pe = cur_pe;
    bool shape = false, simple = false;
    uint32_t n_nrun = 0, plen0 = 0, pp1 = 0;
    if (have) {
      plen0 = cur_hdr; pp1 = pp + 1 + (plen0 + 7) / 8;
      shape = plen0 - (uint32_t)k < 128u && pp1 == pe;
      if (!shape && plen0 - (uint32_t)k < 128u && pp1 < pe) {
        const uint32_t rel = pp1 - cur_pp + (uint32_t)((((uint64_t)(cont + cur_pp)) >> 1) & 1);
        if (rel < 24u) {
          const uint32_t v = (ahead_sel ? ahead0 : ahead1)[rel >> 1];
          shape = __builtin_amdgcn_readfirstlane((rel & 1u) ? v >> 16 : v & 0xFFFFu) == 0;
        }
      }
      if (PIPE && shape) {
        uint32_t n_wd;
        const uint32_t R = front(pp + 1, pp1, 0u, plen0 - (uint32_t)k + 1u, true, n_wd);
        if (R <= MIC_RMAX) { setup(n_wd, 0u, R, N, n_nrun); simple = true; }
      }
    }
    if (PIPE && p_valid) {
      RowAcc acc; acc.label1 = 0; acc.count = 0;
      uint32_t n_ent = 0, overflow = 0, total = 0, cg = MIC_CG_NONE;
      consume(P, acc, n_ent, overflow, total, cg);
      finish(acc, n_ent, total, overflow, r - n_waves, cg);
    } else {
      asm volatile("s_waitcnt vmcnt(0)" ::: "memory");
    }
    if (!have) return false;
    if (!simple) {
      RowAcc acc; acc.label1 = 0; acc.count = 0;
      uint32_t n_ent = 0, overflow = 0, total = 0, cg = MIC_CG_NONE;
      auto chunk = [&](const uint32_t first, const uint32_t cend, const uint32_t base, const uint32_t nk, const bool use_ahead) __attribute__((always_inline)) {
        uint32_t wd;
        const uint32_t R = front(first, cend, base, nk, use_ahead, wd);
        for (uint32_t rbase = 0; rbase < R; rbase += MIC_RMAX) {
          Round L; uint32_t nrun;
          setup(wd, rbase, R, L, nrun);
          issue(L.cur, nrun);
          consume(L, acc, n_ent, overflow, total, cg);
        }
      };
      if (!PIPE && shape) chunk(pp + 1, pp1, 0u, plen0 - (uint32_t)k + 1u, true);
      else {
        bool first_part = true;
        while (pp < pe) {
          uint32_t plen;
          {
            const uint32_t rel = pp - cur_pp + (uint32_t)((((uint64_t)(cont + cur_pp)) >> 1) & 1);
            if (first_part) plen = cur_hdr;
            else if (rel < 24u) {
              const uint32_t v = (ahead_sel ? ahead0 : ahead1)[rel >> 1];
              plen = __builtin_amdgcn_readfirstlane((rel & 1u) ? v >> 16 : v & 0xFFFFu);
            } else plen = __builtin_amdgcn_readfirstlane((uint32_t)cont[pp]);
          }
          const bool ahead_ok = first_part;
          first_part = false;
          if (plen == 0) break;
          const uint32_t first = pp + 1;
          pp = first + (plen + 7) / 8;
          if (plen < (uint32_t)k) continue;
          const uint32_t nk = plen - k + 1;
          const uint32_t cend = pp;
          for (uint32_t base = 0; base < nk; base += 128) chunk(first, cend, base, nk, ahead_ok && base == 0);
        }
      }
      finish(acc, n_ent, total, overflow, r, cg);
    }
    uint32_t t_hdr, t_pp, t_pe;
    __builtin_amdgcn_wave_barrier();
    ahead_take(ahead_sel ? ahead1 : ahead0, n_pp, t_hdr, t_pp, t_pe);
    __builtin_amdgcn_wave_barrier();
    ahead_issue(ahead_sel ? ahead0 : ahead1, t_pp, r + 3 * n_waves);
    ahead_sel ^= 1;
    cur_pp = n_pp; cur_pe = n_pe; cur_hdr = t_hdr; n_pp = t_pp; n_pe = t_pe;
    p_valid = simple;
    if (simple) issue(N.cur, n_nrun);
    r += n_waves;
    return true;
  };
  Round Ra, Rb;
  while (step(Ra, Rb) && step(Rb, Ra)) {}
}

__global__ void __launch_bounds__(256) crowd_finish_kernel(const MicQueryArgs a) {
  const int lane = threadIdx.x & 63;
  const uint32_t wave0 = __builtin_amdgcn_readfirstlane(blockIdx.x * 4 + (threadIdx.x >> 6)), n_waves = gridDim.x * 4;
  const uint32_t* __restrict__ cw = a.crowd;
  const uint32_t pcap = a.crowd_pend_cap;
  uint32_t np = cw[0];
  np = np < pcap ? np : pcap;
  const uint32_t* __restrict__ pend = cw + MIC_CROWD_HDR;
  const uint32_t* __restrict__ items = a.crowd_items;
  const uint32_t* __restrict__ pool = a.crowd_pool;
  const uint4* __restrict__ side = a.t.side;
  const uint32_t smask = a.t.side_mask;
  const int k = a.t.k, ctx = k - a.t.m;
  for (uint32_t p = wave0; p < np; p += n_waves) {
    const uint4 h = *(const uint4*)(pend + 8 * (size_t)p);
    const uint32_t r = __builtin_amdgcn_readfirstlane(h.x), meta = __builtin_amdgcn_readfirstlane(h.z), off = __builtin_amdgcn_readfirstlane(h.w);
    uint32_t total = __builtin_amdgcn_readfirstlane(h.y);
    uint32_t g = __builtin_amdgcn_readfirstlane(pend[8 * (size_t)p + 4]);
    if (meta == 0xFFFFFFFFu) continue;
    uint32_t n_ent = meta & 0xFFu, overflow = (meta >> 8) & 1u;
    RowAcc acc; acc.label1 = 0; acc.count = 0;
    if ((uint32_t)lane < n_ent) { const uint2 e = *(const uint2*)(pool + off + 2 * lane); acc.label1 = e.x; acc.count = e.y; }
    while (g != MIC_CG_NONE) {
      const uint32_t ib = g & 0x7FFFFFFu, n_c = (g >> 27) + 1u;
      g = __builtin_amdgcn_readfirstlane(items[8 * (size_t)ib + 4]);
      for (uint32_t b = 0; b < n_c; b += 4) {
        const uint32_t idx = b + ((uint32_t)lane >> 4);
        const bool valid = idx < n_c;
        uint4 it = make_uint4(0, 0, 0, 0);
        if (valid) it = *(const uint4*)(items + 8 * (size_t)(ib + idx));
        const int jmin = (int)(it.w & 0xFFu), jmax = (int)((it.w >> 8) & 0xFFu);
        int j = jmin + (lane & 15);
        bool go = valid && j <= jmax;
        j = go ? j : jmin;
        const uint64_t K = s_extract(it.x, it.y, it.z, ctx - j, k);
        uint32_t hsh = s_side_hash(K, smask), got = 0;
        while (wballot(go)) {
          uint4 c = make_uint4(0, 0, 0, 0);
          if (go) c = load_slot_quarter(side + hsh);
          if (go) {
            if (c.z == 0) go = false;
            else if (c.x == (uint32_t)K && c.y == (uint32_t)(K >> 32)) { got = c.z; go = false; }
            else hsh = (hsh + 1) & smask;
          }
        }
        tally2(got, 0u, acc, n_ent, overflow, total, lane);
      }
    }
    finish_read(acc, n_ent, total, overflow, r, a, lane);
  }
}


__global__ void merge_rows_kernel(const uint32_t* __restrict__ ra, const uint32_t* __restrict__ rb,
                                  uint32_t* __restrict__ out, uint32_t row_words, size_t n,
                                  uint32_t* __restrict__ results) {
  size_t i = (size_t)blockIdx.x * blockDim.x + threadIdx.x;
  if (i >= n) return;
  const uint32_t* a = ra + i * row_words; const uint32_t* b = rb + i * row_words; uint32_t* o = out + i * row_words;
  uint32_t na = a[0], nb = b[0], ia = 0, ib = 0, no = 0;
  bool ok = na != MIC_ROW_INVALID && nb != MIC_ROW_INVALID;
  if (!ok) { na = 0; nb = 0; }
  while (ia < na || ib < nb) {
    uint32_t va = ia < na ? a[1 + ia] : 0xFFFFFFFFu, vb = ib < nb ? b[1 + ib] : 0xFFFFFFFFu;
    uint32_t ta = ia < na ? (va & 0xFFFF) : 0x10000u, tb = ib < nb ? (vb & 0xFFFF) : 0x10000u;
    uint32_t tgt, cnt;
    if (ta < tb) { tgt = ta; cnt = va >> 16; ++ia; }
    else if (tb < ta) { tgt = tb; cnt = vb >> 16; ++ib; }
    else { tgt = ta; cnt = (va >> 16) + (vb >> 16); ++ia; ++ib; }
    if (no + 1 < row_words && cnt <= 0xFFFF) o[1 + no] = (cnt << 16) | tgt; else ok = false;
    ++no;
  }
  o[0] = ok ? no : MIC_ROW_INVALID;
  (void)results;
}

__global__ void result_rows_kernel(const uint32_t* __restrict__ rows, uint32_t row_words,
                                   uint32_t* __restrict__ results, size_t n) {
  size_t i = (size_t)blockIdx.x * blockDim.x + threadIdx.x;
  if (i >= n) return;
  const uint32_t* row = rows + i * row_words;
// ... 155 lines not shown
    if (rows) {
      uint32_t* orow = rows + (size_t)r * row_words;
      bool fits = nz <= row_words - 1;
      if (fits) {
        uint32_t no = 0;
        for (uint32_t tg = 0; tg < n_targets && fits; ++tg) {
          uint32_t c = row[tg];
          if (!c) continue;
          if (c > 0xFFFF) { fits = false; break; }
          orow[1 + no++] = (c << 16) | tg;
        }
        if (fits) orow[0] = nz;
      }
      if (!fits) { orow[0] = MIC_ROW_INVALID; flags |= MIC_FLAG_ROW_OVERFLOW_; }
    }
    uint4* out = (uint4*)(results + (size_t)r * 8);
    out[0] = make_uint4(sum, best ? 0x10000u - (uint32_t)(best & 0xFFFF) : 0, (uint32_t)(best >> 16),
                        second ? 0x10000u - (uint32_t)(second & 0xFFFF) : 0);
    out[1] = make_uint4((uint32_t)(second >> 16), nz, flags, 0);
  }
}

template <bool KEY64>
__global__ void __launch_bounds__(256) probe_stats_kernel(const MicTable t, const uint32_t* __restrict__ reads_ptr,
                                                          const uint16_t* __restrict__ cont, uint32_t n_reads,
                                                          unsigned long long* __restrict__ out) {
  uint32_t r = blockIdx.x * blockDim.x + threadIdx.x;
  unsigned long long nk = 0, np = 0, nh = 0, nb = 0;
  if (r < n_reads) {
    uint32_t pp = reads_ptr[r];
    const uint32_t pe = reads_ptr[r + 1];
    const int k = t.k;
    const uint64_t cutoff = k == 32 ? ~0ULL : ((1ULL << (2 * k)) - 1);
    while (pp < pe) {
      const uint32_t plen = cont[pp];
      if (plen == 0) break;
      const uint32_t first = pp + 1;
      pp = first + (plen + 7) / 8;
      uint64_t kmer = 0;
      for (uint32_t i = 0; i < plen; ++i) {
        uint32_t nt = (cont[first + i / 8] >> (14 - 2 * (i % 8))) & 3u;
        kmer = ((kmer << 2) | nt) & cutoff;
        if (i + 1 < (uint32_t)k) continue;
        ++nk;
        uint64_t c = canonical(kmer, k);
        uint64_t q = mic_div(c, t.div);
        uint64_t rem = c - q * t.div.d;
        if (rem < t.shard_start || rem >= t.shard_end) continue;
        bool mine = true;
        const bool hit = probe_any<KEY64>(t, kmer, i + 1 - (uint32_t)k, &mine) != 0;
        if (!mine) continue;
        ++np;
        nb += t.layout ? (t.sizes ? t.sizes[rem - t.shard_start] : 0)
                                               : (t.slots[(rem - t.shard_start) * 4].w & 0xFF);
        nh += hit;
      }
    }
  }
  for (int off = 32; off > 0; off >>= 1) {
    nk += __shfl_down(nk, off); np += __shfl_down(np, off); nh += __shfl_down(nh, off); nb += __shfl_down(nb, off);
  }
  if ((threadIdx.x & 63) == 0) { atomicAdd(&out[0], nk); atomicAdd(&out[1], np); atomicAdd(&out[2], nh); atomicAdd(&out[3], nb); }
}

}

hipError_t mic_launch_probe_stats(const MicTable& t, int slot_class, const uint32_t* reads_ptr, const uint16_t* cont,
                                  size_t n_reads, unsigned long long* d_out, hipStream_t s) {
  if (!n_reads) return hipSuccess;
  unsigned blocks = (unsigned)((n_reads + 255) / 256);
  if (slot_class == 64) probe_stats_kernel<true><<<blocks, 256, 0, s>>>(t, reads_ptr, cont, (uint32_t)n_reads, d_out);
  else probe_stats_kernel<false><<<blocks, 256, 0, s>>>(t, reads_ptr, cont, (uint32_t)n_reads, d_out);
  return hipGetLastError();
}

static bool per_kmer_env() { static const bool v = getenv("MIC_S_PER_KMER") != nullptr; return v; }

__global__ void kernels_warm_kernel(uint32_t* p) { if (p && threadIdx.x == 1000) *p = 0; }
hipError_t mic_kernels_warm(hipStream_t s) {
  kernels_warm_kernel<<<1, 64, 0, s>>>(nullptr);
  return hipGetLastError();
}

hipError_t mic_launch_query(const MicQueryArgs& a_in, int slot_class, int n_cu, hipStream_t s) {
  if (a_in.n_reads == 0) return hipSuccess;
  MicQueryArgs a = a_in;
  if (a.crowd) if (const char* e = getenv("MIC_CROWD_CAP")) {
    const long v = atol(e);
    if (v >= 0) {
      if ((uint32_t)v < a.crowd_pend_cap) a.crowd_pend_cap = (uint32_t)v;
      if ((uint32_t)v < a.crowd_item_cap) a.crowd_item_cap = (uint32_t)v;
      if ((uint32_t)v < a.crowd_pool_cap) a.crowd_pool_cap = (uint32_t)v;
    }
  }
  unsigned blocks = (a.n_reads + 3) / 4;
  static int per_cu = [] { const char* e = getenv("MIC_BLOCKS_PER_CU"); int v = e ? atoi(e) : 0; return v > 0 ? v : 256; }();
  unsigned cap = (unsigned)n_cu * (unsigned)per_cu;
  if (blocks > cap) blocks = cap;
  {
    const unsigned fill = (unsigned)n_cu * 8u;
    static const bool grid_dbg = getenv("MIC_GRID_DEBUG") != nullptr;
    unsigned rpw = 8;
    if (grid_dbg) if (const char* e = getenv("MIC_READS_PER_WAVE")) { const int v = atoi(e); if (v > 0) rpw = (unsigned)v; }
    const unsigned by_work = (unsigned)((a.n_reads + 4 * rpw - 1) / (4 * rpw));
    unsigned want = by_work > fill ? by_work : fill;
    if (blocks > want) blocks = want;
  }
  if (const char* e = getenv("MIC_QUERY_BLOCKS")) { const int v = atoi(e); if (v > 0 && (unsigned)v < blocks) blocks = (unsigned)v; }
  if (a.t.layout == 2) {
    const unsigned g = (blocks * 4 + MIC_M_WPB - 1) / MIC_M_WPB, b = 64 * MIC_M_WPB;
    static const bool generic = getenv("MIC_S_GENERIC") != nullptr;
    const bool pt = a.t.parted != 0, fw = a.t.fwd != 0;
    const bool sh = a.t.sharded != 0 || (pt && (per_kmer_env() || (!fw && !(2 * a.t.k - a.t.m > 32 && 2 * a.t.k - a.t.m <= 48))));
    const bool per_kmer = per_kmer_env();
    const bool run_ok = 2 * a.t.k - a.t.m > 32 && 2 * a.t.k - a.t.m <= 48;
    static const unsigned extra_lds = [] { const char* e = getenv("MIC_EXTRA_LDS"); return e ? (unsigned)atoi(e) : 0u; }();
    const bool crowd = a.t.side != nullptr && a.crowd != nullptr;
    bool ran_r = false;
    if (crowd) { const hipError_t ce = hipMemsetAsync(a.crowd, 0, MIC_CROWD_HDR * 4, s); if (ce != hipSuccess) return ce; }
#define LAUNCH_R(KK_, MM_, FW_) do { \
      if (pt) query_kernel_r<KK_, MM_, FW_, true><<<g, b, extra_lds, s>>>(a); else query_kernel_r<KK_, MM_, FW_, false><<<g, b, extra_lds, s>>>(a); \
      ran_r = true; } while (0)
#define LAUNCH_S(KK_, MM_) do { \
      if (fw && !sh && !per_kmer) LAUNCH_R(KK_, MM_, true); \
      else if (!fw && !sh && !per_kmer && run_ok) LAUNCH_R(KK_, MM_, false); \
      else if (fw) { if (sh) query_kernel_s<KK_, MM_, true, true><<<g, b, 0, s>>>(a); else query_kernel_s<KK_, MM_, false, true><<<g, b, 0, s>>>(a); } \
      else { if (sh) query_kernel_s<KK_, MM_, true, false><<<g, b, 0, s>>>(a); else query_kernel_s<KK_, MM_, false, false><<<g, b, 0, s>>>(a); } } while (0)
    if (!generic && a.t.k == 31 && a.t.m == 20) LAUNCH_S(31, 20);
    else if (!generic && a.t.k == 27 && a.t.m == 20) LAUNCH_S(27, 20);
    else if (!generic && a.t.k == 32 && a.t.m == 20) LAUNCH_S(32, 20);
    else LAUNCH_S(0, 0);
#undef LAUNCH_S
#undef LAUNCH_R
    if (ran_r && crowd) {
      const unsigned most = a.n_reads < a.crowd_pend_cap ? a.n_reads : a.crowd_pend_cap;
      unsigned cg = (most + 3) / 4, ccap = (unsigned)n_cu * 16u;
      if (cg > ccap) cg = ccap;
      if (cg) crowd_finish_kernel<<<cg, 256, 0, s>>>(a);
    }
  }
  else if (a.t.layout) {
    {
      const unsigned g = (blocks * 4 + MIC_M_WPB - 1) / MIC_M_WPB, b = 64 * MIC_M_WPB;
      if (MIC_SPEC && a.t.k == 31 && a.t.m == 20) query_kernel_m<31, 20><<<g, b, 0, s>>>(a);
      else if (MIC_SPEC && a.t.k == 27 && a.t.m == 20) query_kernel_m<27, 20><<<g, b, 0, s>>>(a);
      else query_kernel_m<0, 0><<<g, b, 0, s>>>(a);
    }
  }
  else if (slot_class == 64) query_kernel<true><<<blocks, 256, 0, s>>>(a);
  else query_kernel<false><<<blocks, 256, 0, s>>>(a);
  return hipGetLastError();
}

int mic_query_kernel_name(const MicTable& t, int slot_class, char* buf, size_t cap) {
  if (t.layout == 2) {
    static const bool generic = getenv("MIC_S_GENERIC") != nullptr;
    const bool pt = t.parted != 0, fw = t.fwd != 0, per_kmer = per_kmer_env();
    const bool run_ok = 2 * t.k - t.m > 32 && 2 * t.k - t.m <= 48;
    const bool sh = t.sharded != 0 || (pt && (per_kmer || (!fw && !run_ok)));
    const bool spec = !generic && t.m == 20 && (t.k == 31 || t.k == 27 || t.k == 32);
    const int kk = spec ? t.k : 0, mm = spec ? t.m : 0;
    const char* b[2] = {"false", "true"};
    if (!sh && !per_kmer && (fw || run_ok))
      return snprintf(buf, cap, "query_kernel_r<%d, %d, %s, %s>", kk, mm, b[fw], b[pt]);
    return snprintf(buf, cap, "query_kernel_s<%d, %d, %s, %s>", kk, mm, b[sh], b[fw]);
  }
  if (t.layout) {
    const bool spec = MIC_SPEC && t.m == 20 && (t.k == 31 || t.k == 27);
    return snprintf(buf, cap, "query_kernel_m<%d, %d>", spec ? t.k : 0, spec ? t.m : 0);
  }
  return snprintf(buf, cap, "query_kernel<%s>", slot_class == 64 ? "true" : "false");
}

hipError_t mic_launch_merge_rows(const uint32_t* a, const uint32_t* b, uint32_t* out, uint32_t row_words, size_t n,
                                 uint32_t* flags_results, hipStream_t s) {
  if (!n) return hipSuccess;
  merge_rows_kernel<<<(unsigned)((n + 255) / 256), 256, 0, s>>>(a, b, out, row_words, n, flags_results);
  return hipGetLastError();
}

hipError_t mic_launch_result_from_rows(const uint32_t* rows, uint32_t row_words, uint32_t* results, size_t n,
                                       hipStream_t s) {
  if (!n) return hipSuccess;
  result_rows_kernel<<<(unsigned)((n + 255) / 256), 256, 0, s>>>(rows, row_words, results, n);
  return hipGetLastError();
}

// ... 18 lines not shown
```

cuclark_amd/db.py:

```python
import ctypes as C

import numpy as np

from . import _lib
from ._lib import MicConfig, MicDbInfo, MicError, check, MIC_RESULT_WORDS


class MiClarkUnsupported(RuntimeError):
    """mic_gz_*: an input the device path does not take (MIC_E_UNSUPPORTED); the caller uses its other path."""


def _as_np(ptr, shape, dtype):
    n = int(np.prod(shape))
    if n == 0:
        return np.zeros(shape, dtype)
    buf = (C.c_char * (n * np.dtype(dtype).itemsize)).from_address(ptr)
    return np.frombuffer(buf, dtype=dtype).reshape(shape)


class MiClarkDB:
    def __init__(self, k, num_targets, num_batches=1, device=-1, row_words=16, layout=0):
        self.L = _lib.load()
        self.k = int(k)
        self.num_targets = int(num_targets)
# ... 315 lines not shown

    def rollup_device(self, d_rows, d_norm, n_reads, d_rollup, d_levels=0, d_counts=0, filt=None, stream=0):
        from . import host
        f = filt if filt is not None else host.abund_filter()
        check(self.L.mic_rollup_device(self.h, d_rows, d_norm or None, n_reads, C.byref(f), d_rollup, d_levels or None, d_counts or None,
                                       stream or None))

    def rollup_dense_device(self, d_dense, d_ids, n_ids, d_norm, d_rollup, d_levels=0, d_counts=0, filt=None, stream=0):
        from . import host
        f = filt if filt is not None else host.abund_filter()
        check(self.L.mic_rollup_dense_device(self.h, d_dense, d_ids or None, n_ids, d_norm or None, C.byref(f), d_rollup, d_levels or None,
                                             d_counts or None, stream or None))

    def rollup_start(self, filt=None):
        from . import host
        f = filt if filt is not None else host.abund_filter()
        check(self.L.mic_rollup_start(self.h, C.byref(f)))

    def rollup_fetch(self):
        out = np.zeros(self.rollup_layout()[1], np.uint64)
        check(self.L.mic_rollup_fetch(self.h, out.ctypes.data, out.size))
        return out

    def rollup_stop(self):
        check(self.L.mic_rollup_stop(self.h))

    def ingest_rollup_rows(self, slot):
        p, n = C.c_void_p(0), C.c_uint64(0)
        check(self.L.mic_ingest_rollup_rows(self.h, slot, C.byref(p), C.byref(n)))
        return _as_np(p.value, (int(n.value), _lib.MIC_ROLLUP_WORDS), np.uint32).copy()

    def ingest_fetch_group_rows(self, slot, part):
        n, rw = C.c_uint64(0), C.c_uint32(0)
        check(self.L.mic_ingest_fetch_group_rows(self.h, slot, part, None, 0, C.byref(n), C.byref(rw)))
        rows = np.zeros((n.value, rw.value), np.uint32)
        check(self.L.mic_ingest_fetch_group_rows(self.h, slot, part, rows.ctypes.data, rows.size, None, None))
        return rows

    def ingest_fetch_packed(self, slot):
        n, m = C.c_uint64(0), C.c_uint64(0)
        check(self.L.mic_ingest_fetch_packed(self.h, slot, None, 0, None, 0, C.byref(n), C.byref(m)))
        rp = np.zeros(n.value + 1, np.uint32)
        ct = np.zeros(max(m.value, 1), np.uint16)
        check(self.L.mic_ingest_fetch_packed(self.h, slot, rp.ctypes.data, rp.size, ct.ctypes.data, ct.size, None, None))
        return rp, ct[: m.value]

    def ingest_free(self):
        self._ingest = None
        check(self.L.mic_ingest_free(self.h))

    def query_device(self, d_reads_pointer, d_containers, n_reads, d_results, d_rows=0, stream=0):
        check(self.L.mic_query_device(self.h, d_reads_pointer, d_containers, n_reads, d_results, d_rows or None,
                                      stream or None))

    def resolve_flagged_device(self, d_reads_pointer, d_containers, d_results, d_rows=0, stream=0):
        n = C.c_size_t(0)
        check(self.L.mic_resolve_flagged_device(self.h, d_reads_pointer, d_containers, d_results, d_rows or None,
                                                stream or None, C.byref(n)))
        return int(n.value)

    def merge_rows_device(self, d_a, d_b, d_out, n_reads, stream=0):
        check(self.L.mic_merge_rows_device(self.h, d_a, d_b, d_out, n_reads, stream or None))

    def result_from_rows_device(self, d_rows, d_results, n_reads, stream=0):
        check(self.L.mic_result_from_rows_device(self.h, d_rows, d_results, n_reads, stream or None))

    def count_dense_device(self, d_reads_pointer, d_containers, d_ids, n_ids, d_counts, stream=0):
        check(self.L.mic_count_dense_device(self.h, d_reads_pointer, d_containers, d_ids or None, n_ids, d_counts,
                                            stream or None))

    def result_from_dense_device(self, d_counts, d_ids, n_ids, d_results, d_rows=0, stream=0):
        check(self.L.mic_result_from_dense_device(self.h, d_counts, d_ids or None, n_ids, d_results, d_rows or None, stream or None))

    def probe_stats_device(self, d_reads_pointer, d_containers, n_reads):
        out = (C.c_uint64 * 4)()
        check(self.L.mic_probe_stats_device(self.h, d_reads_pointer, d_containers, n_reads, out))
        return dict(kmers=int(out[0]), probed=int(out[1]), hits=int(out[2]), bucket_len_sum=int(out[3]))

    def last_query_ms(self):
        ms = C.c_float(0)
        check(self.L.mic_last_query_ms(self.h, C.byref(ms)))
        return float(ms.value)

    def last_crowd_stats(self):
        out = (C.c_uint32 * 4)()
        check(self.L.mic_last_crowd_stats(self.h, out))
        return dict(reads=int(out[0]), runs=int(out[1]), row_words=int(out[2]), reads_to_dense_path=int(out[3]))
```

include/mi_clark.h:

```cpp
#ifndef MI_CLARK_H
#define MI_CLARK_H

#include <stddef.h>
#include <stdint.h>

#ifdef __cplusplus
extern "C" {
#endif

#define MIC_OK 0
#define MIC_E_INVALID (-1)
#define MIC_E_IO (-2)
#define MIC_E_NOMEM (-3)
#define MIC_E_HIP (-4)
#define MIC_E_STATE (-5)
#define MIC_E_NODEVICE (-6)
#define MIC_E_UNSUPPORTED (-7)

#define MIC_RESULT_WORDS 8
#define MIC_FLAG_ROW_OVERFLOW 1u
#define MIC_FLAG_DENSE_PATH 2u

#define MIC_ROW_INVALID 0xFFFFFFFFu
#define MIC_MAX_PART 65528u
// ... 13 lines not shown
#define MIC_LAYOUT_DIRECT 1
#define MIC_LAYOUT_MINIMIZER 2
#define MIC_LAYOUT_SUPER 3
#define MIC_LAYOUT_SUPER2 4

typedef struct mic_db_info {
  uint64_t htsize;
  uint64_t shard_start;
  uint64_t shard_end;
  uint64_t n_elems;
  uint64_t n_elems_file;
  uint64_t n_slots;
  uint64_t n_overflow;
  uint64_t hbm_bytes;
  int32_t key_bytes;
  int32_t slot_class;
  uint32_t max_bucket;
  uint32_t sampling;
  int32_t layout;
  int32_t minimizer_len;
  uint32_t max_chain;
  uint32_t reserved;
  uint64_t n_entries;
  uint32_t part, n_parts;
  uint64_t part_slot_lo;
  uint64_t part_slot_hi;
  uint64_t n_slots_whole;
  uint64_t side_kmers;
  uint64_t side_bytes;
} mic_db_info;

int mic_create(const mic_config* cfg, mic_engine** out);
int mic_destroy(mic_engine* e);
int mic_debug_stream_pool(uint32_t out[4]);
const char* mic_last_error(void);
int mic_device_count(int* count);

int mic_db_load_files(mic_engine* e, const char* prefix, int key_bytes, uint32_t sampling, uint64_t shard_start,
                      uint64_t shard_end);
int mic_db_load_host(mic_engine* e, const uint8_t* sizes, uint64_t htsize, const void* keys, int key_bytes,
                     const uint16_t* labels, uint32_t sampling, uint64_t shard_start, uint64_t shard_end);
int mic_db_load_device(mic_engine* e, const uint8_t* d_sizes, uint64_t htsize, const void* d_keys, int key_bytes,
                       const uint16_t* d_labels, uint32_t sampling, uint64_t shard_start, uint64_t shard_end);
int mic_db_set_part(mic_engine* e, uint32_t part, uint32_t n_parts);
int mic_db_reserve_hbm(mic_engine* e, uint64_t bytes);
int mic_peer_matrix(int* matrix, int n_devices);
int mic_device_memory(int device, uint64_t* free_bytes, uint64_t* total_bytes);
int mic_db_load_files_multi(mic_engine* const* engines, size_t n_engines, const char* prefix, int key_bytes, uint32_t sampling);
int mic_db_kernel_name(const mic_engine* e, char* buf, size_t cap);
int mic_db_get_info(const mic_engine* e, mic_db_info* info);
int mic_db_unload(mic_engine* e);
const char* mic_db_last_build_report(void);

int mic_batches_alloc(mic_engine* e, size_t num_reads_total, size_t max_reads, size_t max_containers,
                      const uint32_t* index_batches, int extended, uint32_t** results, uint32_t** rows,
                      uint32_t** reads_pointer , uint16_t** containers );
int mic_batch_ready(mic_engine* e, size_t batch, size_t n_reads, size_t n_containers);
int mic_batch_query(mic_engine* e, size_t batch, int extended, int followup);
int mic_batch_wait(mic_engine* e, size_t batch);
int mic_batch_dense_counts(mic_engine* e, size_t batch, size_t read_in_batch, uint32_t* counts);
int mic_batch_check(mic_engine* e, size_t batch, int* done);
int mic_batch_merge_shards(mic_engine* const* engines, size_t n_engines, size_t batch);
int mic_batch_query_group(mic_engine* const* engines, size_t n_engines, size_t batch, int extended);
int mic_sync(mic_engine* e);
int mic_thread_bind_near_device(mic_engine* e, int on);
int mic_batches_free(mic_engine* e);

int mic_query_device(mic_engine* e, const uint32_t* d_reads_pointer, const uint16_t* d_containers, size_t n_reads,
                     uint32_t* d_results, uint32_t* d_rows, void* stream);
int mic_resolve_flagged_device(mic_engine* e, const uint32_t* d_reads_pointer, const uint16_t* d_containers,
                               uint32_t* d_results, uint32_t* d_rows, void* stream, size_t* n_resolved);
int mic_merge_rows_device(mic_engine* e, const uint32_t* d_rows_a, const uint32_t* d_rows_b, uint32_t* d_rows_out,
                          size_t n_reads, void* stream);
int mic_result_from_rows_device(mic_engine* e, const uint32_t* d_rows, uint32_t* d_results, size_t n_reads,
                                void* stream);
int mic_count_dense_device(mic_engine* e, const uint32_t* d_reads_pointer, const uint16_t* d_containers,
                           const uint32_t* d_read_ids, size_t n_ids, uint32_t* d_counts, void* stream);
int mic_result_from_dense_device(mic_engine* e, const uint32_t* d_counts, const uint32_t* d_ids, size_t n_ids,
                                 uint32_t* d_results, uint32_t* d_rows, void* stream);
int mic_probe_stats_device(mic_engine* e, const uint32_t* d_reads_pointer, const uint16_t* d_containers, size_t n_reads,
                           uint64_t out[4]);
int mic_last_query_ms(mic_engine* e, float* ms);
int mic_last_crowd_stats(mic_engine* e, uint32_t out[4]);
int mic_debug_fetch_crowd(mic_engine* e, uint32_t* out, size_t words, uint32_t caps[3]);

#define MIC_INGEST_PAIRED 1
#define MIC_INGEST_FASTQ_2LINE 2
#define MIC_INGEST_RESIDENT 4
#define MIC_INGEST_RESIDENT_FASTQ 12
#define MIC_INGEST_NO_CSV 16
#define MIC_INGEST_OK 0u
#define MIC_INGEST_FALLBACK 1u
#define MIC_INGEST_ODD_RECORD 2u
#define MIC_INGEST_TRUNCATED 4u
#define MIC_INGEST_LONG_READ 8u
#define MIC_INGEST_TOO_MANY 16u
#define MIC_INGEST_DENSE 32u

typedef struct mic_ingest_result {
  uint64_t n_reads;
  uint64_t csv_bytes;
  const char* csv;
  const uint32_t* results;
  uint32_t status;
  uint32_t n_lines;
} mic_ingest_result;

int mic_ingest_alloc(mic_engine* e, size_t n_slots, size_t max_bytes, const char* const* target_names, uint32_t n_targets,
                     int want_results, uint8_t** raw );
int mic_ingest_classify(mic_engine* e, size_t slot, size_t n_bytes, int flags, mic_ingest_result* out);
int mic_ingest_classify_group(mic_engine* const* group, size_t n_group, size_t owner, size_t slot, size_t n_bytes, int flags,
                              mic_ingest_result* out);
int mic_ingest_fetch_packed(mic_engine* e, size_t slot, uint32_t* reads_pointer, size_t rp_cap, uint16_t* containers,
                            size_t cont_cap, uint64_t* n_reads, uint64_t* n_containers);
int mic_ingest_fetch_group_rows(mic_engine* owner, size_t slot, size_t part, uint32_t* rows, size_t cap_words, uint64_t* n_reads,
                                uint32_t* row_words);
#define MIC_GROUP_STATS_FIELDS 10
int mic_ingest_group_stats(mic_engine* owner, double* out, size_t cap);
int mic_ingest_free(mic_engine* e);
int mic_gz_inflate_device(mic_engine* e, const void* gz, size_t gz_bytes, void** d_text, size_t* n_text, uint32_t* crc32_expected);
int mic_gz_copy_text(mic_engine* e, const void* d_text, size_t offset, size_t n, void* host_dst);
int mic_gz_free_text(mic_engine* e, void* d_text);
int mic_gz_reserve(mic_engine* e, size_t gz_bytes, uint32_t isize);
uint64_t mic_gz_reserve_bytes(size_t gz_bytes, uint32_t isize);
int mic_gz_release(mic_engine* e);
typedef struct mic_gz_stream mic_gz_stream;
int mic_gz_stream_open(mic_engine* e, const void* gz, size_t gz_bytes, uint32_t stripes, mic_gz_stream** out, void** d_text, size_t* n_text);
int mic_gz_stream_next(mic_gz_stream* s, size_t* n_final, int* done);
int mic_gz_stream_close(mic_gz_stream* s, int keep_text);

#define MIC_PAIRS_LINES 1u
#define MIC_PAIRS_HEADER 2u
#define MIC_PAIRS_ID 4u
#define MIC_PAIRS_BIG 8u
typedef struct mic_pairs mic_pairs;
int mic_pairs_index_device(mic_engine* e, const void* d_text1, size_t n1, const void* d_text2, size_t n2, mic_pairs** out,
                           uint64_t* n_records, uint32_t* status);
int mic_pairs_offsets(const mic_pairs* p, const uint64_t** samples, size_t* n_samples, uint32_t* stride);
int mic_pairs_merge_to_slot(mic_engine* e, mic_pairs* p, uint64_t r0, uint64_t r1, size_t slot, size_t* n_bytes);
int mic_pairs_text(mic_engine* e, mic_pairs* p, uint64_t r0, uint64_t r1, void* host_dst, size_t cap, size_t* n_bytes);
int mic_pairs_free(mic_engine* e, mic_pairs* p);

typedef struct mic_text mic_text;
int mic_text_index_device(mic_engine* e, const void* d_text, size_t n, mic_text** out, uint64_t* n_records, uint32_t* status);
int mic_text_index_front_device(mic_engine* e, const void* d_text, size_t n, mic_text** out, uint64_t* n_records, uint64_t* n_used, uint32_t* status);
int mic_text_format(const mic_text* p);
int mic_text_offsets(const mic_text* p, const uint64_t** samples, size_t* n_samples, uint32_t* stride);
int mic_text_to_slot(mic_engine* e, mic_text* p, uint64_t r0, uint64_t r1, size_t slot, size_t* n_bytes);
int mic_text_copy(mic_engine* e, mic_text* p, uint64_t r0, uint64_t r1, void* host_dst, size_t cap, size_t* n_bytes);
int mic_text_free(mic_engine* e, mic_text* p);

typedef struct mic_abund_filter {
  uint64_t conf_num, conf_den;
  uint64_t gamma_num, gamma_den;
} mic_abund_filter;
int mic_abundance_start(mic_engine* e, const mic_abund_filter* filter);
int mic_abundance_fetch(mic_engine* e, uint64_t* counts, size_t n);
int mic_abundance_stop(mic_engine* e);
int mic_abundance_device(mic_engine* e, const uint32_t* d_results, const uint32_t* d_norm, size_t n_reads, const mic_abund_filter* filter,
                         uint64_t* d_counts, void* stream);
int mic_abundance_host(const uint32_t* results, const uint32_t* norm, size_t n_reads, int k, uint32_t n_targets,
                       const mic_abund_filter* filter, uint64_t* counts);
int mic_abund_parse(const char* text, uint32_t max_int, uint64_t* num, uint64_t* den);

#define MIC_ROLLUP_WORDS 8
#define MIC_ROLLUP_MAX_LEVELS 7
// ... 71 lines not shown
```

Before: 1924.

## Process two reads per wave in paired halves of the run-query kernel

Adds a paired mode to the run-based query kernel in which each wave classifies two reads at once, one per 32-lane half. It stages run slots for both reads, tallies per-half label counts with DPP reductions, and prefetches both reads' headers and offsets together. Reads whose run count or row size does not fit fall back to the plain per-read path. The aim is to raise lane utilisation and amortise per-read latency on short reads, at the cost of more LDS per block, possibly lower occupancy, and extra fallback work, plus new counters for diagnostics.

```diff
diff --git a/cuclark_amd/_lib.py b/cuclark_amd/_lib.py
--- a/cuclark_amd/_lib.py
+++ b/cuclark_amd/_lib.py
@@ -95,6 +95,7 @@
     ("mic_probe_stats_device", C.c_int, [_VP, _VP, _VP, _SZ, C.POINTER(C.c_uint64)]),
     ("mic_last_query_ms", C.c_int, [_VP, C.POINTER(C.c_float)]),
     ("mic_last_crowd_stats", C.c_int, [_VP, C.POINTER(C.c_uint32)]),
+    ("mic_last_pair_stats", C.c_int, [_VP, C.POINTER(C.c_uint32)]),
     ("mic_debug_fetch_crowd", C.c_int, [_VP, _VP, _SZ, C.POINTER(C.c_uint32)]),
     ("mic_debug_stream_pool", C.c_int, [C.POINTER(C.c_uint32)]),
     ("mic_ingest_alloc", C.c_int, [_VP, _SZ, _SZ, C.POINTER(C.c_char_p), C.c_uint32, C.c_int, C.POINTER(_VP)]),
@@ -206,7 +207,12 @@
                           "(there is no CPU fallback for the k-mer query path)")
     lib = C.CDLL(LIB_PATH)
     for name, res, args in SYMBOLS:
-        fn = getattr(lib, name)
+        try:
+            fn = getattr(lib, name)
+        except AttributeError:
+            if os.environ.get("MIC_LIB_PATH") and name == "mic_last_pair_stats":
+                continue
+            raise
         fn.restype = res
         fn.argtypes = args
     _lib = lib
diff --git a/cuclark_amd/csrc/mic_engine.hip b/cuclark_amd/csrc/mic_engine.hip
--- a/cuclark_amd/csrc/mic_engine.hip
+++ b/cuclark_amd/csrc/mic_engine.hip
@@ -142,7 +142,7 @@
   uint32_t* h_results = nullptr; uint32_t* h_rows = nullptr;
   size_t num_reads_total = 0;
   std::mutex submit_mu;
-  uint32_t* d_flagged = nullptr; uint32_t flagged_cap = 0;
+  uint32_t* d_flagged = nullptr; uint32_t* d_flagged_base = nullptr; uint32_t flagged_cap = 0;
   uint32_t* d_crowd = nullptr; size_t crowd_reads = 0;
   hipEvent_t ev0 = nullptr, ev1 = nullptr;
   bool timed = false;
@@ -636,7 +636,8 @@
   if (he == hipSuccess) he = mic_stream_get(&e->down_stream);
   if (he == hipSuccess) he = mic_event_get(&e->ev0, true);
   if (he == hipSuccess) he = mic_event_get(&e->ev1, true);
-  if (he == hipSuccess) he = hipMalloc(&e->d_flagged, (size_t)(kFlaggedCap + 1) * 4);
+  if (he == hipSuccess) he = hipMalloc(&e->d_flagged_base, (size_t)(4 + kFlaggedCap + 1) * 4);
+  if (he == hipSuccess) e->d_flagged = e->d_flagged_base + 4;
   if (he != hipSuccess) { mic_destroy(e); return fail(MIC_E_HIP, "engine setup: %s", hipGetErrorString(he)); }
   e->flagged_cap = kFlaggedCap;
   *out = e;
@@ -653,7 +654,7 @@
   if (e->slots) hipFree(e->slots);
   if (e->side) hipFree(e->side);
   if (e->d_sizes) hipFree(e->d_sizes);
-  if (e->d_flagged) hipFree(e->d_flagged);
+  if (e->d_flagged_base) hipFree(e->d_flagged_base);
   if (e->d_crowd) hipFree(e->d_crowd);
   if (e->abund.d_counts) hipFree(e->abund.d_counts);
   if (e->rollup.d_counts) hipFree(e->rollup.d_counts);
@@ -1271,11 +1272,12 @@
   int rc = set_device(e);
   if (rc) return rc;
   hipStream_t s = stream ? (hipStream_t)stream : e->stream;
-  HIPTRY(hipMemsetAsync(e->d_flagged, 0, 4, s));
+  HIPTRY(hipMemsetAsync(e->d_flagged_base, 0, 20, s));
   MicQueryArgs a;
   a.t = e->table; a.reads_ptr = d_rp; a.cont = d_cont; a.n_reads = (uint32_t)n_reads;
   a.row_words = e->cfg.row_words; a.results = d_results; a.rows = d_rows;
   a.flagged = e->d_flagged; a.flagged_cap = e->flagged_cap;
+  a.pair_stat = e->d_flagged_base;
   if (e->table.side && n_reads > e->crowd_reads) {
     HIPTRY(hipStreamSynchronize(s));
     if (e->d_crowd) { hipFree(e->d_crowd); e->d_crowd = nullptr; e->crowd_reads = 0; }
@@ -1307,6 +1309,18 @@
   if (rc) return rc;
   HIPTRY(hipEventSynchronize(e->ev1));
   HIPTRY(hipMemcpy(out, e->d_crowd, 16, hipMemcpyDeviceToHost));
+  return MIC_OK;
+}
+
+int mic_last_pair_stats(mic_engine* e, uint32_t out[4]) {
+  if (!e || !out) return fail(MIC_E_INVALID, "null argument");
+  out[0] = out[1] = out[2] = out[3] = 0;
+  if (!e->timed) return MIC_OK;
+  int rc = set_device(e);
+  if (rc) return rc;
+  HIPTRY(hipEventSynchronize(e->ev1));
+  out[3] = mic_query_pairs(e->table, e->last_n_reads);
+  if (out[3]) HIPTRY(hipMemcpy(out, e->d_flagged_base, 12, hipMemcpyDeviceToHost));
   return MIC_OK;
 }
 
diff --git a/cuclark_amd/csrc/mic_internal.h b/cuclark_amd/csrc/mic_internal.h
--- a/cuclark_amd/csrc/mic_internal.h
+++ b/cuclark_amd/csrc/mic_internal.h
@@ -89,6 +89,8 @@
   uint32_t* crowd;
   uint32_t* crowd_items; uint32_t* crowd_pool;
   uint32_t crowd_pend_cap, crowd_item_cap, crowd_pool_cap;
+  uint32_t* pair_stat = nullptr;
+  uint32_t pair_runs = 0;
 };
 
 #define MIC_CROWD_HDR 8
@@ -116,6 +118,7 @@
 extern thread_local uint64_t mic_build_reserved_hbm;
 
 hipError_t mic_launch_query(const MicQueryArgs& a, int slot_class, int n_cu, hipStream_t s);
+uint32_t mic_query_pairs(const MicTable& t, size_t n_reads);
 int mic_query_kernel_name(const MicTable& t, int slot_class, char* buf, size_t cap);
 hipError_t mic_kernels_warm(hipStream_t s);
 hipError_t mic_launch_merge_rows(const uint32_t* a, const uint32_t* b, uint32_t* out, uint32_t row_words, size_t n,
diff --git a/cuclark_amd/csrc/mic_kernels.hip b/cuclark_amd/csrc/mic_kernels.hip
--- a/cuclark_amd/csrc/mic_kernels.hip
+++ b/cuclark_amd/csrc/mic_kernels.hip
@@ -2,6 +2,7 @@
 #include "mic_device.h"
 
 #include <stdlib.h>
+#include <type_traits>
 
 #ifndef MIC_EXP
 #define MIC_EXP 0
@@ -314,6 +315,15 @@
 #ifndef MIC_R_PIPE
 #define MIC_R_PIPE 2
 #endif
+#ifndef MIC_R_PAIR
+#define MIC_R_PAIR 1
+#endif
+#ifndef MIC_R_PAIR_C
+#define MIC_R_PAIR_C 24
+#endif
+static_assert(MIC_R_PAIR_C % 8 == 0 && MIC_R_PAIR_C >= 16 && MIC_R_PAIR_C <= 32, "eight slots per LDS-DMA instruction; the plain road stages 32 slots; a half has 32 lanes");
+constexpr bool mic_r_pipe(int kk, bool fwd) { return kk != 0 && (MIC_R_PIPE >= 2 || (MIC_R_PIPE == 1 && fwd)); }
+constexpr bool mic_r_pair(int kk, bool fwd) { return MIC_R_PAIR != 0 && mic_r_pipe(kk, fwd); }
 __device__ __forceinline__ uint32_t staged_at(uint32_t i) { return i * MIC_MSTRIDE + (i >> 3) * MIC_R_SKEW; }
 #ifndef MIC_M_SKEW
 #define MIC_M_SKEW 0
@@ -986,16 +996,61 @@
   }
 }
 
+struct RunTally {
+  uint32_t n_ent[2], total[2], cg[2], overflow, full;
+};
+
+__device__ __forceinline__ void tally_counts2(uint32_t lab1, uint32_t cnt, RowAcc& acc, RunTally& T, int lane) {
+  uint64_t mm = wballot(lab1 != 0);
+  while (mm) {
+    const uint32_t mlo = (uint32_t)mm, mhi = (uint32_t)(mm >> 32);
+    const uint32_t lA = mlo ? __builtin_amdgcn_readlane(lab1, __builtin_ctz(mlo)) : 0u;
+    const uint32_t lB = mhi ? __builtin_amdgcn_readlane(lab1, 32 + __builtin_ctz(mhi)) : 0u;
+    const uint32_t l1 = lane < 32 ? lA : lB;
+    const bool mine = lab1 == l1;
+    mm &= ~wballot(mine);
+    uint32_t v = mine ? cnt : 0u;
+    v += (uint32_t)__builtin_amdgcn_update_dpp(0, (int)v, 0x111, 0xF, 0xF, true);
+    v += (uint32_t)__builtin_amdgcn_update_dpp(0, (int)v, 0x112, 0xF, 0xF, true);
+    v += (uint32_t)__builtin_amdgcn_update_dpp(0, (int)v, 0x114, 0xF, 0xF, true);
+    v += (uint32_t)__builtin_amdgcn_update_dpp(0, (int)v, 0x118, 0xF, 0xF, true);
+    const uint32_t sA = __builtin_amdgcn_readlane(v, 15) + __builtin_amdgcn_readlane(v, 31);
+    const uint32_t sB = __builtin_amdgcn_readlane(v, 47) + __builtin_amdgcn_readlane(v, 63);
+    T.total[0] += sA; T.total[1] += sB;
+    const uint32_t sum = lane < 32 ? sA : sB;
+    const bool hit = l1 != 0 && acc.label1 == l1;
+    const uint64_t f = wballot(hit);
+    if (hit) acc.count += sum;
+    const bool newA = lA != 0 && (uint32_t)f == 0, newB = lB != 0 && (uint32_t)(f >> 32) == 0;
+    if (newA || newB) {
+      if ((newA && T.n_ent[0] >= 32u) || (newB && T.n_ent[1] >= 32u)) T.full = 1;
+      else {
+        const uint32_t at = lane < 32 ? (newA ? T.n_ent[0] : 64u) : (newB ? 32u + T.n_ent[1] : 64u);
+        if ((uint32_t)lane == at) { acc.label1 = l1; acc.count = sum; }
+        T.n_ent[0] += newA ? 1u : 0u; T.n_ent[1] += newB ? 1u : 0u;
+      }
+    }
+  }
+}
+
+constexpr int mic_r_stage_slots(bool pair) { return pair ? 2 * MIC_R_PAIR_C : MIC_RMAX; }
+constexpr int mic_r_stage_u4(bool pair) { return mic_r_stage_slots(pair) * MIC_MSTRIDE + (mic_r_stage_slots(pair) / 8 - 1) * MIC_R_SKEW; }
+constexpr int mic_r_lds_bytes(bool pair) { return MIC_M_WPB * (mic_r_stage_u4(pair) * 16 + (pair ? 2 : 1) * 264 + 512) + 64 + 32; }
+constexpr int mic_r_blocks_per_cu(bool pair) {
+  return !pair ? 32 / MIC_M_WPB : (163840 / mic_r_lds_bytes(true) < 32 / MIC_M_WPB ? 163840 / mic_r_lds_bytes(true) : 32 / MIC_M_WPB);
+}
+
 template <int KK, int MM, bool FWD, bool PART>
-__global__ void __launch_bounds__(64 * MIC_M_WPB, 32 / MIC_M_WPB) query_kernel_r(const MicQueryArgs a) {
-  __shared__ uint4 s_stage[MIC_M_WPB][MIC_RMAX * MIC_MSTRIDE + (MIC_RMAX / 8 - 1) * MIC_R_SKEW];
-  __shared__ uint16_t s_rec[MIC_M_WPB][132];
-  __shared__ uint32_t s_ahead[MIC_M_WPB][2][64];
+__global__ void __launch_bounds__(64 * MIC_M_WPB, mic_r_blocks_per_cu(mic_r_pair(KK, FWD)) * MIC_M_WPB / 4) query_kernel_r(const MicQueryArgs a) {
+  constexpr bool PAIR = mic_r_pair(KK, FWD);
+  __shared__ uint4 s_stage[MIC_M_WPB][mic_r_stage_u4(PAIR)];
+  __shared__ uint16_t s_rec[MIC_M_WPB][PAIR ? 2 : 1][132];
+  __shared__ uint32_t s_ahead[MIC_M_WPB * 2 * 64 + 16];
   __shared__ uint32_t s_part[PART ? MIC_M_WPB : 1][2];
   const int lane = threadIdx.x & 63;
   const int wv = __builtin_amdgcn_readfirstlane(threadIdx.x >> 6);
   uint4* stage = s_stage[wv];
-  uint16_t* rec = s_rec[wv];
+  uint16_t* rec = s_rec[wv][0];
   const uint32_t wave0 = __builtin_amdgcn_readfirstlane(blockIdx.x * MIC_M_WPB + wv);
   const uint32_t n_waves = gridDim.x * MIC_M_WPB;
   const MicTable& t = a.t;
@@ -1005,8 +1060,8 @@
   const uint16_t* __restrict__ cont = a.cont;
   auto below = [](uint64_t mask) { return (uint32_t)__builtin_amdgcn_mbcnt_hi((uint32_t)(mask >> 32), __builtin_amdgcn_mbcnt_lo((uint32_t)mask, 0u)); };
 
-  uint32_t* ahead0 = s_ahead[wv][0];
-  uint32_t* ahead1 = s_ahead[wv][1];
+  uint32_t* ahead0 = s_ahead + wv * 128;
+  uint32_t* ahead1 = ahead0 + 64;
   auto ahead_issue = [&](uint32_t* entry, uint32_t pp_w, uint32_t r_ptr) {
     const uint64_t abase = ((uint64_t)(cont + pp_w)) & ~3ULL;
     const uint32_t rr = r_ptr < a.n_reads ? r_ptr : a.n_reads - 1;
@@ -1035,8 +1090,48 @@
     const uint32_t up = (uint32_t)__builtin_amdgcn_update_dpp(0, (int)raw, 0x101, 0xF, 0xF, true);
     return __builtin_amdgcn_perm(up, raw, odd ? 0x05040706u : 0x03020504u);
   };
-  uint32_t cur_pp, cur_pe, cur_hdr, n_pp, n_pe, ahead_sel;
-  {
+  const uint32_t n_pairs = (a.n_reads + 1u) >> 1;
+  auto ahead_issue2 = [&](uint32_t* entry, uint32_t ppA, uint32_t ppB, uint32_t j_ptr) {
+    const uint64_t baseA = ((uint64_t)(cont + ppA)) & ~3ULL, baseB = ((uint64_t)(cont + ppB)) & ~3ULL;
+    const uint32_t jc = j_ptr < n_pairs ? j_ptr : n_pairs - 1u;
+    if (lane < 12) {
+      __builtin_amdgcn_global_load_lds((const __attribute__((address_space(1))) void*)((const uint32_t*)baseA + lane),
+                                       (__attribute__((address_space(3))) void*)entry, 4, 0, 0);
+      __builtin_amdgcn_global_load_lds((const __attribute__((address_space(1))) void*)((const uint32_t*)baseB + lane),
+                                       (__attribute__((address_space(3))) void*)(entry + 16), 4, 0, 0);
+    }
+    if (lane < 4) {
+      const uint32_t want = 2u * jc + (((uint32_t)lane + 1u) >> 1), most = a.n_reads - 1u + ((uint32_t)lane & 1u);
+      __builtin_amdgcn_global_load_lds((const __attribute__((address_space(1))) void*)(a.reads_ptr + (want < most ? want : most)),
+                                       (__attribute__((address_space(3))) void*)(entry + 32), 4, 0, 0);
+    }
+  };
+  auto hdr_of = [&](uint32_t first, uint32_t pp_w) {
+    return ((((uint64_t)(cont + pp_w)) >> 1) & 1) ? first >> 16 : first & 0xFFFFu;
+  };
+  auto ahead_take2 = [&](const uint32_t* entry, uint32_t ppA, uint32_t ppB, uint32_t& hdrA, uint32_t& hdrB,
+                         uint32_t& p0, uint32_t& p1, uint32_t& p2, uint32_t& p3) {
+    const uint32_t raw = entry[lane];
+    p0 = __builtin_amdgcn_readlane(raw, 32); p1 = __builtin_amdgcn_readlane(raw, 33);
+    p2 = __builtin_amdgcn_readlane(raw, 34); p3 = __builtin_amdgcn_readlane(raw, 35);
+    hdrA = hdr_of(__builtin_amdgcn_readlane(raw, 0), ppA);
+    hdrB = hdr_of(__builtin_amdgcn_readlane(raw, 16), ppB);
+  };
+  uint32_t cur_pp = 0, cur_pe = 0, cur_hdr = 0, n_pp = 0, n_pe = 0, ahead_sel;
+  uint32_t cpA = 0, ceA = 0, cpB = 0, ceB = 0, chA = 0, chB = 0, npA = 0, neA = 0, npB = 0, neB = 0;
+  if constexpr (PAIR) {
+    const uint32_t r0 = 2u * (wave0 < n_pairs ? wave0 : n_pairs - 1u), nr = a.n_reads;
+    cpA = __builtin_amdgcn_readfirstlane(a.reads_ptr[r0]);
+    ceA = __builtin_amdgcn_readfirstlane(a.reads_ptr[r0 + 1u]);
+    cpB = __builtin_amdgcn_readfirstlane(a.reads_ptr[r0 + 1u < nr ? r0 + 1u : nr - 1u]);
+    ceB = __builtin_amdgcn_readfirstlane(a.reads_ptr[r0 + 2u < nr ? r0 + 2u : nr]);
+    ahead_issue2(ahead0, cpA, cpB, wave0 + n_waves);
+    asm volatile("s_waitcnt vmcnt(0)" ::: "memory");
+    __builtin_amdgcn_wave_barrier();
+    ahead_take2(ahead0, cpA, cpB, chA, chB, npA, neA, npB, neB);
+    ahead_issue2(ahead1, npA, npB, wave0 + 2 * n_waves);
+    ahead_sel = 1;
+  } else {
     const uint32_t r0 = wave0 < a.n_reads ? wave0 : a.n_reads - 1;
     cur_pp = __builtin_amdgcn_readfirstlane(a.reads_ptr[r0]); cur_pe = __builtin_amdgcn_readfirstlane(a.reads_ptr[r0 + 1]);
     ahead_issue(ahead0, cur_pp, wave0 + n_waves);
@@ -1046,15 +1141,16 @@
     ahead_issue(ahead1, n_pp, wave0 + 2 * n_waves);
     ahead_sel = 1;
   }
-  constexpr bool PIPE = KK != 0 && (MIC_R_PIPE >= 2 || (MIC_R_PIPE == 1 && FWD));
+  constexpr bool PIPE = mic_r_pipe(KK, FWD);
   struct Round {
     uint32_t G0, G1, G2, cur;
     int jmax, jmin, remaining;
   };
-  auto front = [&](const uint32_t first, const uint32_t cend, const uint32_t base, const uint32_t nk, const bool use_ahead, uint32_t& wd_out) __attribute__((always_inline)) -> uint32_t {
+  auto front = [&](const uint32_t first, const uint32_t cend, const uint32_t base, const uint32_t nk, const bool use_ahead,
+                   const uint32_t* aent, const uint32_t app, uint16_t* rec, uint32_t& wd_out) __attribute__((always_inline)) -> uint32_t {
     int ln = lane;
     asm volatile("" : "+v"(ln));
-    const uint32_t wd = use_ahead ? ahead_word(ahead_sel ? ahead0 : ahead1, cur_pp)
+    const uint32_t wd = use_ahead ? ahead_word(aent, app)
                                   : window_word_w(cont, first, cend, base, ln, false, 0u);
     wd_out = wd;
     const uint32_t n_act = nk - base < 128u ? nk - base : 128u;
@@ -1089,18 +1185,19 @@
       lo = (uint32_t)x; hi = (uint32_t)(x >> 32);
     }
   };
-  auto setup = [&](const uint32_t wd, const uint32_t rbase, const uint32_t R, Round& L, uint32_t& nrun_out) __attribute__((always_inline)) {
-    const uint32_t nrun = R - rbase < MIC_RMAX ? R - rbase : MIC_RMAX;
+  auto setup = [&](auto paired, const uint32_t wd, const uint32_t rbase, const uint32_t R, const uint32_t RB, Round& L, uint32_t& nrun_out) __attribute__((always_inline)) {
+    constexpr bool P2 = decltype(paired)::value;
+    const uint32_t nrun = P2 ? R : (R - rbase < MIC_RMAX ? R - rbase : MIC_RMAX);
     nrun_out = nrun;
-    const bool vr = (uint32_t)lane < nrun;
-    const uint32_t ri = vr ? rbase + (uint32_t)lane : 0u;
+    const bool vr = P2 ? (uint32_t)(lane & 31) < (lane < 32 ? R : RB) : (uint32_t)lane < nrun;
+    const uint32_t ri = vr ? (P2 ? (uint32_t)(lane & 31) + (lane < 32 ? 0u : 132u) : rbase + (uint32_t)lane) : 0u;
     const uint32_t rc0 = rec[ri], rc1 = rec[ri + 1];
     const int qa = (int)(rc0 & 255u), i0 = (int)(rc0 >> 8);
     const int n = (int)(rc1 >> 8) - i0;
     const int s1 = qa - ctx - 1;
     const int D = s1 >> 4;
     const uint32_t tsh = 30u - 2u * (uint32_t)(s1 & 15);
-    const int a0 = D << 2;
+    const int a0 = P2 ? (D << 2) + ((lane & 32) << 2) : D << 2;
     const uint32_t W0 = (uint32_t)__builtin_amdgcn_ds_bpermute(a0, (int)wd), W1 = (uint32_t)__builtin_amdgcn_ds_bpermute(a0 + 4, (int)wd),
                    W2 = (uint32_t)__builtin_amdgcn_ds_bpermute(a0 + 8, (int)wd), W3 = (uint32_t)__builtin_amdgcn_ds_bpermute(a0 + 12, (int)wd);
     uint32_t G0 = __builtin_amdgcn_alignbit(W0, W1, tsh), G1 = __builtin_amdgcn_alignbit(W1, W2, tsh), G2 = __builtin_amdgcn_alignbit(W2, W3, tsh);
@@ -1152,7 +1249,28 @@
                                          (__attribute__((address_space(3))) void*)(uintptr_t)(so + 16u * (64 + MIC_R_SKEW) * (uint32_t)i), 16, 0, 0);
     }
   };
-  auto consume = [&](Round& L, RowAcc& acc, uint32_t& n_ent, uint32_t& overflow, uint32_t& total, uint32_t& cg) __attribute__((always_inline)) {
+  const uint32_t sl2 = (uint32_t)(lane & 31) + (lane < 32 ? 0u : (uint32_t)MIC_R_PAIR_C);
+  auto issue2 = [&](const uint32_t cur, const uint32_t nrA, const uint32_t nrB) __attribute__((always_inline)) {
+    constexpr int NG = 2 * MIC_R_PAIR_C / 8;
+    uint32_t sidx[NG];
+    __builtin_amdgcn_wave_barrier();
+    if ((lane & 31) < MIC_R_PAIR_C) ((uint32_t*)stage)[sl2] = cur;
+    __builtin_amdgcn_wave_barrier();
+    uint32_t so = (uint32_t)(uintptr_t)(__attribute__((address_space(3))) void*)stage;
+    asm volatile("" : "+s"(so));
+#pragma unroll
+    for (int i = 0; i < NG; ++i) sidx[i] = ((const uint32_t*)stage)[8 * i + (lane >> 3)];
+#pragma unroll
+    for (int i = 0; i < NG; ++i) {
+      if (8u * i >= MIC_R_PAIR_C + nrB) break;
+      if (8u * i >= nrA && 8u * i + 8u <= MIC_R_PAIR_C) continue;
+      if (sidx[i] != 0xFFFFFFFFu)
+        __builtin_amdgcn_global_load_lds((const __attribute__((address_space(1))) void*)(slots + (uint64_t)sidx[i] * 8 + (lane & 7)),
+                                         (__attribute__((address_space(3))) void*)(uintptr_t)(so + 16u * (64 + MIC_R_SKEW) * (uint32_t)i), 16, 0, 0);
+    }
+  };
+  auto consume = [&](auto paired, Round& L, RowAcc& acc, RunTally& T) __attribute__((always_inline)) {
+    constexpr bool P2 = decltype(paired)::value;
     const uint32_t G0 = L.G0, G1 = L.G1, G2 = L.G2;
     uint32_t key, xhi_;
     region_x(G0, G1, key, xhi_);
@@ -1161,12 +1279,12 @@
     int remaining = L.remaining;
     bool again = false;
     do {
-      if (again) issue(cur, MIC_RMAX);
+      if (again) { if constexpr (P2) issue2(cur, MIC_R_PAIR_C, MIC_R_PAIR_C); else issue(cur, MIC_RMAX); }
       again = true;
       asm volatile("s_waitcnt vmcnt(0)" ::: "memory");
       __builtin_amdgcn_wave_barrier();
       const bool vl = cur != 0xFFFFFFFFu;
-      const uint32_t* q = (const uint32_t*)(stage + (vl ? staged_at((uint32_t)lane) : 0));
+      const uint32_t* q = (const uint32_t*)(stage + (vl ? staged_at(P2 ? sl2 : (uint32_t)lane) : 0));
       const uint4 ka = *(const uint4*)q;
       const uint2 kb = *(const uint2*)(q + 4);
       uint32_t e = (ka.x < key) + (ka.y < key) + (ka.z < key) + (ka.w < key) + (kb.x < key) + (kb.y < key);
@@ -1195,7 +1313,8 @@
         remaining = (same && mineq && (pl >> 16) == 0) ? MIC_R_CROWDED : remaining;
 #endif
         const uint32_t lab_new = (pl & 0xFFFFu) + 1u;
-        tally_counts(hits ? lab_new : 0u, hits, acc, n_ent, overflow, total, lane);
+        if constexpr (P2) tally_counts2(hits ? lab_new : 0u, hits, acc, T, lane);
+        else tally_counts(hits ? lab_new : 0u, hits, acc, T.n_ent[0], T.overflow, T.total[0], lane);
         remaining -= (int)hits;
         more = same && remaining > 0 && e < 5;
         e += more ? 1u : 0u;
@@ -1205,9 +1324,14 @@
       cur = 0xFFFFFFFFu;
       if (wballot(nx)) { if (nx && q[5] <= key) cur = q[31]; }
     } while (wballot(cur != 0xFFFFFFFFu));
-    if (!(MIC_X & 2) && __builtin_expect(wballot(remaining <= MIC_R_CROWDED) != 0, 0)) {
-      const bool crowded = remaining <= MIC_R_CROWDED;
-      const uint32_t n_c = (uint32_t)__popcll(wballot(crowded));
+    if (!(MIC_X & 2) && __builtin_expect(wballot(remaining <= MIC_R_CROWDED) != 0, 0) && !(P2 && T.full)) {
+#pragma nounroll
+      for (int h = 0; h < (P2 ? 2 : 1); ++h) {
+      const bool crowded = remaining <= MIC_R_CROWDED && (!P2 || (lane >> 5) == h);
+      const uint64_t cmask = wballot(crowded);
+      if (!cmask) continue;
+      uint32_t cg = h ? T.cg[1] : T.cg[0];
+      const uint32_t n_c = (uint32_t)__popcll(cmask);
       uint64_t kpv = (uint64_t)__builtin_amdgcn_kernarg_segment_ptr();
       asm volatile("" : "+v"(kpv));
       const MicQueryArgs* kv = (const MicQueryArgs*)kpv;
@@ -1223,11 +1347,13 @@
       asm volatile("" : "+v"(ib));
       const bool room = ib <= icap && n_c <= icap - ib;
       if (crowded && room) {
-        uint32_t* it = itb + 8 * ((size_t)ib + below(wballot(crowded)));
+        uint32_t* it = itb + 8 * ((size_t)ib + below(cmask));
         it[0] = G0; it[1] = G1; it[2] = G2; it[3] = (uint32_t)jmin | ((uint32_t)jmax << 8);
         it[4] = cg;
       }
       cg = __builtin_amdgcn_readfirstlane(room ? (ib | ((n_c - 1u) << 27)) : MIC_CG_DENSE);
+      if (h) T.cg[1] = cg; else T.cg[0] = cg;
+      }
     }
   };
   auto finish = [&](const RowAcc& acc, uint32_t n_ent, uint32_t total, uint32_t overflow, uint32_t r, const uint32_t cg) __attribute__((always_inline)) {
@@ -1286,30 +1412,30 @@
       }
       if (PIPE && shape) {
         uint32_t n_wd;
-        const uint32_t R = front(pp + 1, pp1, 0u, plen0 - (uint32_t)k + 1u, true, n_wd);
-        if (R <= MIC_RMAX) { setup(n_wd, 0u, R, N, n_nrun); simple = true; }
+        const uint32_t R = front(pp + 1, pp1, 0u, plen0 - (uint32_t)k + 1u, true, ahead_sel ? ahead0 : ahead1, cur_pp, rec, n_wd);
+        if (R <= MIC_RMAX) { setup(std::false_type{}, n_wd, 0u, R, 0u, N, n_nrun); simple = true; }
       }
     }
     if (PIPE && p_valid) {
       RowAcc acc; acc.label1 = 0; acc.count = 0;
-      uint32_t n_ent = 0, overflow = 0, total = 0, cg = MIC_CG_NONE;
-      consume(P, acc, n_ent, overflow, total, cg);
-      finish(acc, n_ent, total, overflow, r - n_waves, cg);
+      RunTally T = {{0, 0}, {0, 0}, {MIC_CG_NONE, MIC_CG_NONE}, 0, 0};
+      consume(std::false_type{}, P, acc, T);
+      finish(acc, T.n_ent[0], T.total[0], T.overflow, r - n_waves, T.cg[0]);
     } else {
       asm volatile("s_waitcnt vmcnt(0)" ::: "memory");
     }
     if (!have) return false;
     if (!simple) {
       RowAcc acc; acc.label1 = 0; acc.count = 0;
-      uint32_t n_ent = 0, overflow = 0, total = 0, cg = MIC_CG_NONE;
+      RunTally T = {{0, 0}, {0, 0}, {MIC_CG_NONE, MIC_CG_NONE}, 0, 0};
       auto chunk = [&](const uint32_t first, const uint32_t cend, const uint32_t base, const uint32_t nk, const bool use_ahead) __attribute__((always_inline)) {
         uint32_t wd;
-        const uint32_t R = front(first, cend, base, nk, use_ahead, wd);
+        const uint32_t R = front(first, cend, base, nk, use_ahead, ahead_sel ? ahead0 : ahead1, cur_pp, rec, wd);
         for (uint32_t rbase = 0; rbase < R; rbase += MIC_RMAX) {
           Round L; uint32_t nrun;
-          setup(wd, rbase, R, L, nrun);
+          setup(std::false_type{}, wd, rbase, R, 0u, L, nrun);
           issue(L.cur, nrun);
-          consume(L, acc, n_ent, overflow, total, cg);
+          consume(std::false_type{}, L, acc, T);
         }
       };
       if (!PIPE && shape) chunk(pp + 1, pp1, 0u, plen0 - (uint32_t)k + 1u, true);
@@ -1336,7 +1462,7 @@
           for (uint32_t base = 0; base < nk; base += 128) chunk(first, cend, base, nk, ahead_ok && base == 0);
         }
       }
-      finish(acc, n_ent, total, overflow, r, cg);
+      finish(acc, T.n_ent[0], T.total[0], T.overflow, r, T.cg[0]);
     }
     uint32_t t_hdr, t_pp, t_pe;
     __builtin_amdgcn_wave_barrier();
@@ -1350,8 +1476,156 @@
     r += n_waves;
     return true;
   };
+
+  const uint32_t lim = a.pair_runs < (uint32_t)MIC_R_PAIR_C ? a.pair_runs : (uint32_t)MIC_R_PAIR_C;
+  auto shape_of = [&](const uint32_t* ent, const uint32_t pp, const uint32_t pe, const uint32_t hdr, uint32_t& pp1) -> bool {
+    pp1 = pp + 1 + (hdr + 7) / 8;
+    bool shape = hdr - (uint32_t)k < 128u && pp1 == pe;
+    if (!shape && hdr - (uint32_t)k < 128u && pp1 < pe) {
+      const uint32_t rel = pp1 - pp + (uint32_t)((((uint64_t)(cont + pp)) >> 1) & 1);
+      if (rel < 24u) {
+        const uint32_t v = ent[rel >> 1];
+        shape = __builtin_amdgcn_readfirstlane((rel & 1u) ? v >> 16 : v & 0xFFFFu) == 0;
+      }
+    }
+    return shape;
+  };
+  auto plain_read = [&](const uint32_t rr, const uint32_t pp0, const uint32_t pe, const uint32_t hdr, const bool has_ent,
+                        const uint32_t* ent) __attribute__((always_inline)) {
+    RowAcc acc; acc.label1 = 0; acc.count = 0;
+    RunTally T = {{0, 0}, {0, 0}, {MIC_CG_NONE, MIC_CG_NONE}, 0, 0};
+    bool first_part = true;
+    uint32_t pp = pp0;
+    while (pp < pe) {
+      uint32_t plen;
+      const uint32_t rel = pp - pp0 + (uint32_t)((((uint64_t)(cont + pp0)) >> 1) & 1);
+      if (first_part) plen = hdr;
+      else if (has_ent && rel < 24u) {
+        const uint32_t v = ent[rel >> 1];
+        plen = __builtin_amdgcn_readfirstlane((rel & 1u) ? v >> 16 : v & 0xFFFFu);
+      } else plen = __builtin_amdgcn_readfirstlane((uint32_t)cont[pp]);
+      const bool ahead_ok = first_part && has_ent;
+      first_part = false;
+      if (plen == 0) break;
+      const uint32_t first = pp + 1;
+      pp = first + (plen + 7) / 8;
+      if (plen < (uint32_t)k) continue;
+      const uint32_t nk = plen - k + 1;
+      const uint32_t cend = pp;
+      for (uint32_t base = 0; base < nk; base += 128) {
+        uint32_t wd;
+        const uint32_t R = front(first, cend, base, nk, ahead_ok && base == 0, ent, pp0, rec, wd);
+        for (uint32_t rbase = 0; rbase < R; rbase += MIC_RMAX) {
+          Round L; uint32_t nrun;
+          setup(std::false_type{}, wd, rbase, R, 0u, L, nrun);
+          issue(L.cur, nrun);
+          consume(std::false_type{}, L, acc, T);
+        }
+      }
+    }
+    finish(acc, T.n_ent[0], T.total[0], T.overflow, rr, T.cg[0]);
+  };
+  auto finish2 = [&](const RowAcc& acc, const RunTally& T, const uint32_t rA, const bool haveB) __attribute__((always_inline)) {
+    const bool hb = lane >= 32;
+    const uint32_t nv = hb ? T.n_ent[1] : T.n_ent[0];
+    const bool big = (lane & 31) == 0 && acc.count > 0xFFFFu;
+    if ((T.cg[0] & T.cg[1]) == MIC_CG_NONE && (T.n_ent[0] | T.n_ent[1]) <= 1u && (a.rows == nullptr || a.row_words >= 2u) && !wballot(big)) {
+      if ((lane & 31) == 0 && (!hb || haveB)) {
+        const uint32_t r = rA + (hb ? 1u : 0u);
+        uint4 lo, hi;
+        lo.x = hb ? T.total[1] : T.total[0]; lo.y = acc.label1; lo.z = acc.count; lo.w = 0;
+        hi.x = 0; hi.y = nv; hi.z = 0; hi.w = 0;
+        uint4* out = (uint4*)(a.results + (size_t)r * 8);
+        out[0] = lo; out[1] = hi;
+        if (a.rows) {
+          uint32_t* row = a.rows + (size_t)r * a.row_words;
+          row[0] = nv;
+          if (nv) row[1] = (acc.count << 16) | (acc.label1 - 1u);
+        }
+      }
+    } else {
+      const uint32_t ul = bperm((lane + 32) & 63, acc.label1), uc = bperm((lane + 32) & 63, acc.count);
+#pragma nounroll
+      for (int h = 0; h < 2; ++h) {
+        if (h && !haveB) break;
+        RowAcc x;
+        x.label1 = h ? ul : acc.label1; x.count = h ? uc : acc.count;
+        finish(x, h ? T.n_ent[1] : T.n_ent[0], h ? T.total[1] : T.total[0], 0u, rA + (uint32_t)h, h ? T.cg[1] : T.cg[0]);
+      }
+    }
+  };
+  uint32_t pj = wave0;
+  auto step2 = [&](Round& P, Round& N) __attribute__((always_inline)) -> bool {
+    const bool have = pj < n_pairs;
+    const uint32_t rA = 2u * pj;
+    const bool haveB = have && rA + 1u < a.n_reads;
+    const uint32_t* ent = ahead_sel ? ahead0 : ahead1;
+    bool formed = false;
+    uint32_t nrA = 0, nrB = 0, why = 2;
+    if (have) {
+      uint32_t pp1A, pp1B = 0;
+      const bool shA = shape_of(ent, cpA, ceA, chA, pp1A);
+      const bool shB = !haveB || shape_of(ent + 16, cpB, ceB, chB, pp1B);
+      if (shA && shB) {
+        uint32_t wdA, wdB = 0, RB = 0;
+        const uint32_t RA = front(cpA + 1, pp1A, 0u, chA - (uint32_t)k + 1u, true, ent, cpA, rec, wdA);
+        if (haveB) RB = front(cpB + 1, pp1B, 0u, chB - (uint32_t)k + 1u, true, ent + 16, cpB, rec + 132, wdB);
+        if (RA <= lim && RB <= lim) {
+          const uint32_t up = bperm(lane & 31, wdB);
+          uint32_t dummy;
+          setup(std::true_type{}, lane < 32 ? wdA : up, 0u, RA, RB, N, dummy);
+          nrA = RA; nrB = RB; formed = true;
+        } else why = 1;
+      }
+    }
+    uint32_t todo = 0;
+    if (p_valid) {
+      RowAcc acc; acc.label1 = 0; acc.count = 0;
+      RunTally T = {{0, 0}, {0, 0}, {MIC_CG_NONE, MIC_CG_NONE}, 0, 0};
+      consume(std::true_type{}, P, acc, T);
+      const uint32_t prA = 2u * (pj - n_waves);
+      const bool pB = prA + 1u < a.n_reads;
+      if (__builtin_expect(T.full != 0, 0)) {
+        todo = pB ? 3u : 1u;
+        if (a.pair_stat != nullptr && lane == 0) atomicAdd(a.pair_stat, 1u);
+      } else finish2(acc, T, prA, pB);
+    } else {
+      asm volatile("s_waitcnt vmcnt(0)" ::: "memory");
+    }
+    if (have && !formed) {
+      todo |= haveB ? 12u : 4u;
+      if (a.pair_stat != nullptr && lane == 0) atomicAdd(a.pair_stat + why, 1u);
+    }
+    if (todo) {
+#pragma nounroll
+      for (uint32_t q = 0; q < 4; ++q) {
+        if (!((todo >> q) & 1u)) continue;
+        if (q < 2) {
+          const uint32_t rr = 2u * (pj - n_waves) + q;
+          const uint32_t pp = __builtin_amdgcn_readfirstlane(a.reads_ptr[rr]), pe = __builtin_amdgcn_readfirstlane(a.reads_ptr[rr + 1]);
+          const uint32_t hdr = pp < pe ? __builtin_amdgcn_readfirstlane((uint32_t)cont[pp]) : 0u;
+          plain_read(rr, pp, pe, hdr, false, ent);
+        } else if (q == 2) plain_read(rA, cpA, ceA, chA, true, ent);
+        else plain_read(rA + 1u, cpB, ceB, chB, true, ent + 16);
+      }
+    }
+    if (!have) return false;
+    uint32_t thA, thB, t0, t1, t2, t3;
+    __builtin_amdgcn_wave_barrier();
+    ahead_take2(ahead_sel ? ahead1 : ahead0, npA, npB, thA, thB, t0, t1, t2, t3);
+    __builtin_amdgcn_wave_barrier();
+    ahead_issue2(ahead_sel ? ahead0 : ahead1, t0, t2, pj + 3 * n_waves);
+    ahead_sel ^= 1;
+    cpA = npA; ceA = neA; cpB = npB; ceB = neB; chA = thA; chB = thB;
+    npA = t0; neA = t1; npB = t2; neB = t3;
+    p_valid = formed;
+    if (formed) issue2(N.cur, nrA, nrB);
+    pj += n_waves;
+    return true;
+  };
   Round Ra, Rb;
-  while (step(Ra, Rb) && step(Rb, Ra)) {}
+  if constexpr (PAIR) { while (step2(Ra, Rb) && step2(Rb, Ra)) {} }
+  else { while (step(Ra, Rb) && step(Rb, Ra)) {} }
 }
 
 __global__ void __launch_bounds__(256) crowd_finish_kernel(const MicQueryArgs a) {
@@ -1673,9 +1947,26 @@
   return hipGetLastError();
 }
 
+static bool r_kernel_paired(const MicTable& t) {
+  if (t.layout != 2) return false;
+  static const bool generic = getenv("MIC_S_GENERIC") != nullptr;
+  const bool pt = t.parted != 0, fw = t.fwd != 0, per_kmer = per_kmer_env();
+  const bool run_ok = 2 * t.k - t.m > 32 && 2 * t.k - t.m <= 48;
+  const bool sh = t.sharded != 0 || (pt && (per_kmer || (!fw && !run_ok)));
+  const bool spec = !generic && t.m == 20 && (t.k == 31 || t.k == 27 || t.k == 32);
+  return !sh && !per_kmer && (fw || run_ok) && spec && mic_r_pair(t.k, fw);
+}
+
+uint32_t mic_query_pairs(const MicTable& t, size_t n_reads) { return r_kernel_paired(t) ? (uint32_t)((n_reads + 1) / 2) : 0u; }
+
 hipError_t mic_launch_query(const MicQueryArgs& a_in, int slot_class, int n_cu, hipStream_t s) {
   if (a_in.n_reads == 0) return hipSuccess;
   MicQueryArgs a = a_in;
+  a.pair_runs = MIC_R_PAIR_C;
+  if (const char* e = getenv("MIC_R_PAIR_RUNS")) { const int v = atoi(e); if (v > 0 && v < MIC_R_PAIR_C) a.pair_runs = (uint32_t)v; }
+  const bool pair = r_kernel_paired(a.t);
+  const unsigned units = pair ? (a.n_reads + 1u) / 2u : a.n_reads;
+  const unsigned resident = pair ? (unsigned)mic_r_blocks_per_cu(true) : 8u;
   if (a.crowd) if (const char* e = getenv("MIC_CROWD_CAP")) {
     const long v = atol(e);
     if (v >= 0) {
@@ -1684,16 +1975,17 @@
       if ((uint32_t)v < a.crowd_pool_cap) a.crowd_pool_cap = (uint32_t)v;
     }
   }
-  unsigned blocks = (a.n_reads + 3) / 4;
+  unsigned blocks = (units + 3) / 4;
   static int per_cu = [] { const char* e = getenv("MIC_BLOCKS_PER_CU"); int v = e ? atoi(e) : 0; return v > 0 ? v : 256; }();
   unsigned cap = (unsigned)n_cu * (unsigned)per_cu;
   if (blocks > cap) blocks = cap;
   {
-    const unsigned fill = (unsigned)n_cu * 8u;
+    const unsigned fill = (unsigned)n_cu * resident;
     static const bool grid_dbg = getenv("MIC_GRID_DEBUG") != nullptr;
     unsigned rpw = 8;
     if (grid_dbg) if (const char* e = getenv("MIC_READS_PER_WAVE")) { const int v = atoi(e); if (v > 0) rpw = (unsigned)v; }
-    const unsigned by_work = (unsigned)((a.n_reads + 4 * rpw - 1) / (4 * rpw));
+    if (pair) rpw = rpw > 1 ? rpw / 2 : 1;
+    const unsigned by_work = (unsigned)((units + 4 * rpw - 1) / (4 * rpw));
     unsigned want = by_work > fill ? by_work : fill;
     if (blocks > want) blocks = want;
   }
diff --git a/cuclark_amd/db.py b/cuclark_amd/db.py
--- a/cuclark_amd/db.py
+++ b/cuclark_amd/db.py
@@ -421,6 +421,11 @@
         check(self.L.mic_last_query_ms(self.h, C.byref(ms)))
         return float(ms.value)
 
+    def last_pair_stats(self):
+        out = (C.c_uint32 * 4)()
+        check(self.L.mic_last_pair_stats(self.h, out))
+        return dict(abandoned_row_full=int(out[0]), not_formed_runs=int(out[1]), not_formed_shape=int(out[2]), pairs=int(out[3]))
+
     def last_crowd_stats(self):
         out = (C.c_uint32 * 4)()
         check(self.L.mic_last_crowd_stats(self.h, out))
diff --git a/include/mi_clark.h b/include/mi_clark.h
--- a/include/mi_clark.h
+++ b/include/mi_clark.h
@@ -119,6 +119,7 @@
                            uint64_t out[4]);
 int mic_last_query_ms(mic_engine* e, float* ms);
 int mic_last_crowd_stats(mic_engine* e, uint32_t out[4]);
+int mic_last_pair_stats(mic_engine* e, uint32_t out[4]);
 int mic_debug_fetch_crowd(mic_engine* e, uint32_t* out, size_t words, uint32_t caps[3]);
 
 #define MIC_INGEST_PAIRED 1
```

Measured after the change: 976.6. -49.2%, worse.
